# mrlooi/PoseCNN

Hardware: AMD Instinct MI355X
Metric: frames/sec 640x480x21-class Hough-vote+RoI+ADD-loss, 1/2/4/8 MI355X (higher is better)
Workload: dtype f32 (FC GEMMs: exact 3-way split-bf16 x6 MFMA, products within 2^-24, fp32 accumulate: fp32-faithful)

## Files before the change

include/posecnn_hip.h:

```cpp
#ifndef POSECNN_HIP_H
#define POSECNN_HIP_H

#include <stddef.h>
#include <stdint.h>

#ifdef __cplusplus
extern "C" {
#endif

#define PCNN_OK 0
#define PCNN_EINVAL 1
#define PCNN_EHIP 2
#define PCNN_ECAPACITY 3

#define PCNN_MAX_ROI 128

int pcnn_abi_version(void);
const char* pcnn_strerror(int code);

int pcnn_set_completion_event(void* event);
int pcnn_completion_event_pending(void);

size_t pcnn_hough_voting_workspace_size(int B, int H, int W, int C, int skip_pixels, float vote_thr);

int pcnn_hough_voting(const int32_t* label, const float* vertex, const float* extents, const float* meta,
                      int num_meta, const float* gt, int num_gt, int B, int H, int W, int C, int batch_base,
                      int global_batch, int is_train, float inlier_thr, int label_thr, float vote_thr,
                      float per_thr, int skip_pixels, float* top_box, float* top_pose, float* top_target,
                      float* top_weight, int32_t* top_domain, int32_t* num_rois, int cap, int32_t* debug_counts,
                      void* workspace, size_t workspace_bytes, void* stream);

int pcnn_hough_voting_prob(const float* prob, int32_t* label_out, const float* vertex, const float* extents,
                           const float* meta, int num_meta, const float* gt, int num_gt, int B, int H, int W, int C,
                           int batch_base, int global_batch, int is_train, float inlier_thr, int label_thr,
                           float vote_thr, float per_thr, int skip_pixels, float* top_box, float* top_pose,
                           float* top_target, float* top_weight, int32_t* top_domain, int32_t* num_rois, int cap,
                           int32_t* debug_counts, void* workspace, size_t workspace_bytes, void* stream);

int pcnn_hough_voting_compact(const int32_t* label, const float* vertex3, const float* extents, const float* meta,
                              int num_meta, const float* gt, int num_gt, int B, int H, int W, int C, int batch_base,
                              int global_batch, int is_train, float inlier_thr, int label_thr, float vote_thr,
                              float per_thr, int skip_pixels, float* top_box, float* top_pose, float* top_target,
                              float* top_weight, int32_t* top_domain, int32_t* num_rois, int cap,
                              int32_t* debug_counts, void* workspace, size_t workspace_bytes, void* stream);

int pcnn_hough_voting_grad(float* grad_label, float* grad_vertex, int B, int H, int W, int C, void* stream);

int pcnn_hough_voting_diag(const void* workspace, int B, int H, int W, int C, int skip_pixels, float vote_thr,
                           int32_t* diag_host4, void* stream);

int pcnn_roi_pool_fwd(const float* data, int B, int H, int W, int C, int layout, const float* rois, int R_cap,
                      int roi_stride, int batch_base, const int32_t* num_rois_dev, float spatial_scale, int pooled_h, int pooled_w,
                      int pool_channel, float* top, int32_t* argmax, void* stream);

int pcnn_roi_pool_fwd_accumulate(const float* data, int B, int H, int W, int C, int layout, const float* rois,
                                 int R_cap, int roi_stride, int batch_base, const int32_t* num_rois_dev,
                                 float spatial_scale, int pooled_h, int pooled_w, int pool_channel, float* top,
                                 int32_t* argmax, void* stream);

int pcnn_roi_pool_fwd_pair(const float* data_a, int Ha, int Wa, float scale_a, const float* data_b, int Hb, int Wb,
                           float scale_b, int B, int C, const float* rois, int R_cap, int roi_stride,
                           int batch_base, const int32_t* num_rois_dev, int pooled_h, int pooled_w, float* top_sum,
                           int32_t* argmax_a, int32_t* argmax_b, void* stream);

int pcnn_roi_pool_fwd_pair_px(const float* data_a, int Ha, int Wa, float scale_a, const float* data_b, int Hb,
                              int Wb, float scale_b, int B, int C, const float* rois, int R_cap, int roi_stride,
                              int batch_base, const int32_t* num_rois_dev, int pooled_h, int pooled_w,
                              float* top_sum, uint16_t* argmax_a, uint16_t* argmax_b, void* stream);

size_t pcnn_roi_pool_bwd_workspace_size(int B, int R_cap);

int pcnn_roi_pool_bwd_form(int B, int H, int W, int C, int layout, int pool_channel, int pooled_h, int pooled_w,
                           int R_cap, int px);

int pcnn_roi_pool_bwd(const float* top_diff, const int32_t* argmax, int B, int H, int W, int C, int layout,
                      const float* rois, int R_cap, int roi_stride, int batch_base, const int32_t* num_rois_dev,
                      float spatial_scale, int pooled_h, int pooled_w, int pool_channel, float* bottom_diff,
                      void* workspace, size_t workspace_bytes, void* stream);

int pcnn_roi_pool_bwd_px(const float* top_diff, const uint16_t* argmax_px, int B, int H, int W, int C,
                         const float* rois, int R_cap, int roi_stride, int batch_base, const int32_t* num_rois_dev,
                         float spatial_scale, int pooled_h, int pooled_w, float* bottom_diff, void* workspace,
                         size_t workspace_bytes, void* stream);

size_t pcnn_add_loss_workspace_size(int R_cap, int C, int P);
size_t pcnn_add_loss_stats_offset(int R_cap, int C, int P);

int pcnn_add_loss_fwd(const float* pred, const float* target, const float* weight, const float* points,
                      const float* symmetry, int R_cap, const int32_t* num_rois_dev, int C, int P, float margin,
                      int loss_norm_rows, const int32_t* loss_norm_rows_dev, float* loss, float* bottom_diff,
                      void* workspace, size_t workspace_bytes, void* stream);

int pcnn_add_loss_prep(const float* weight, const float* symmetry, int R_cap, const int32_t* num_rois_dev, int C,
                       int P, void* workspace, size_t workspace_bytes, void* stream);
int pcnn_add_loss_fwd_prepared(const float* pred, const float* target, const float* weight, const float* points,
                               const float* symmetry, int R_cap, const int32_t* num_rois_dev, int C, int P,
                               float margin, int loss_norm_rows, const int32_t* loss_norm_rows_dev, float* loss,
                               float* bottom_diff, void* workspace, size_t workspace_bytes, void* stream);

int pcnn_add_loss_fwd_head_bwd(const float* pred, const float* target, const float* weight, const float* points,
                               const float* symmetry, int R_cap, const int32_t* num_rois_dev, int C, int P,
                               float margin, int loss_norm_rows, const int32_t* loss_norm_rows_dev,
                               float* bottom_diff, void* workspace, size_t workspace_bytes, const float* tanh_out,
                               const float* d_pred_scale, float* d_y8, void* stream);
int pcnn_add_loss_total(int R_cap, const int32_t* num_rois_dev, int C, int P, const void* workspace,
                        size_t workspace_bytes, float* loss, void* stream);

int pcnn_add_loss_bwd(const float* top_diff, const float* bottom_diff, int n, const int32_t* num_rois_dev,
                      int row_len, float* out, void* stream);

int pcnn_div_rn_check(const float* x, float b, int n, int dbl, float* out, void* stream);

int pcnn_backproject_fwd(const float* data, const float* label, const float* depth, const float* meta, int num_meta,
                         const float* label_3d, int B, int H, int W, int Ch, int NC, int grid_size,
                         int kernel_size, float threshold, float* top_data, float* top_label, float* top_flag,
                         void* stream);

int pcnn_backproject_bwd(const float* top_diff, const float* depth, const float* meta, int num_meta, int B, int H,
                         int W, int Ch, int grid_size, float* bottom_diff, void* stream);

size_t pcnn_gemm_workspace_size(int M, int N, int K, int m_dynamic, int precision);

int pcnn_gemm(int M, int N, int K, const float* A, const float* A2, int lda, int a_trans, const float* B, int ldb,
              int b_trans, float* Cm, int ldc, const float* bias, int act, const float* mask, int ldm,
              const int32_t* M_dev, const int32_t* K_dev, int precision, void* workspace, size_t workspace_bytes,
              void* stream);

int pcnn_gemm_drop(int M, int N, int K, const float* A, const float* A2, int lda, int a_trans, const float* B,
                   int ldb, int b_trans, float* Cm, int ldc, const float* bias, int act, const float* mask, int ldm,
                   const uint8_t* drop, int ldd, float keep_prob, const int32_t* M_dev, const int32_t* K_dev,
                   int precision, void* workspace, size_t workspace_bytes, void* stream);

int pcnn_gemm_drop_gen(int M, int N, int K, const float* A, const float* A2, int lda, int a_trans, const float* B,
                       int ldb, int b_trans, float* Cm, int ldc, const float* bias, int act, uint8_t* drop_out,
                       int ldd, float keep_prob, uint64_t seed, const int64_t* step_dev, int stream_id,
                       const int32_t* M_dev, const int32_t* K_dev, int precision, void* workspace,
                       size_t workspace_bytes, void* stream);

size_t pcnn_tp_bytes(int rows, int K);
int pcnn_split_tp(const float* src, long row_stride, long k_stride, int rows, const int32_t* rows_dev, int K,
                  const int32_t* K_dev, void* dst, size_t dst_bytes, void* stream);
int pcnn_gemm_tp(int M, int N, int K, const void* A_tp, const void* B_tp, float* Cm, int ldc, const float* bias,
                 int act, const float* mask, int ldm, const uint8_t* drop, int ldd, float keep_prob,
                 const int32_t* M_dev, const int32_t* K_dev, void* workspace, size_t workspace_bytes, void* stream);

int pcnn_dropout_mask(uint8_t* mask, int rows, int cols, int ld, const int32_t* rows_dev, uint64_t seed,
                      const int64_t* step_dev, int stream_id, float keep_prob, void* stream);

int pcnn_philox_check(const uint32_t* ctr, const uint32_t* key, int n, uint32_t* out, void* stream);

size_t pcnn_pose2d_workspace_size(int H, int W, int C, int n_hyp);
int pcnn_pose2d(const int32_t* label, const float* vertmap, const float* extents, int H, int W, int C, float fx,
                float fy, float px, float py, uint64_t seed, int n_hyp, int max_iter, float* poses_out,
                float* hyps_out, int32_t* hyp_px, int32_t* inl_out, int32_t* final_out, void* workspace,
                size_t workspace_bytes, void* stream);

size_t pcnn_pose3d_workspace_size(int H, int W, int C, int n_hyp);
int pcnn_pose3d(const int32_t* label, const uint16_t* depth, const float* vertmap, const float* extents, int H, int W,
                int C, float fx, float fy, float px, float py, float depth_factor, uint64_t seed, int n_hyp,
                int max_iter, int nm_evals, float* poses_out, float* hyps_out, int32_t* hyp_px, int32_t* inl_out,
                int32_t* final_out, float* energy_out, float* eye_out, void* workspace, size_t workspace_bytes,
                void* stream);

int pcnn_colsum(const float* X, int M, int N, int ldx, const int32_t* M_dev, float* out, void* stream);

int pcnn_pose_head_fwd(const float* y8, const float* poses_weight, int R_cap, const int32_t* num_rois_dev, int D,
                       float* tanh_out, float* pred, void* stream);

int pcnn_pose_head_bwd(const float* d_pred, const float* d_pred_scale, const float* tanh_out,
                       const float* poses_weight, const float* pred, int R_cap, const int32_t* num_rois_dev, int D,
                       float* d_y8, void* stream);

int pcnn_box_nms(const float* rois, int R_cap, int roi_stride, const int32_t* num_rois_dev, float thresh,
                 int32_t* keep, int32_t* num_keep, const float* poses_init, const float* poses_pred, int pred_dim,
                 float* rois_out, float* poses_out, void* stream);

int pcnn_argmax_2d(const float* prob, int B, int H, int W, int C, int32_t* label, void* stream);
int pcnn_hard_label_fwd(const float* prob, const int32_t* gt, int B, int H, int W, int C, float threshold,
                        float* top, void* stream);
int pcnn_hard_label_bwd(float* grad_prob, float* grad_gt, int B, int H, int W, int C, void* stream);

int pcnn_vertex_pred_compact(const float* feat, const float* weights, const float* bias, const int32_t* label, int B,
                             int H, int W, int K, int C, float* vertex3, void* stream);

int pcnn_icp_live_vertices(const uint16_t* depth, const int32_t* label, int H, int W, const int32_t* obj_ids, int L,
                           float factor, float fx, float fy, float px, float py, float* live, void* stream);
size_t pcnn_icp_workspace_size(int N, int H, int W);
int pcnn_icp(const float* live, int num_live, const int32_t* live_index, const float* pred_vertices,
             const float* pred_normals, int N, int H, int W, float fx, float fy, float px, float py, float znear, float zfar, float max_error,
             int iterations, const float* pose_in, float* update, float* pose_out, float* systems, void* workspace,
             size_t workspace_bytes, void* stream);
size_t pcnn_icp_reduce_workspace_size(int L, int H, int W);
int pcnn_icp_center(const float* live, const int32_t* label, const int32_t* obj_ids, int L, const float* vertmap,
                    const float* pred_vertices, const float* pred_normals, int H, int W, float max_error,
                    const float* pose_in, float* out, float* pose_out, void* workspace, size_t workspace_bytes,
                    void* stream);
size_t pcnn_energy_records_workspace_size(int N, int H, int W);
int pcnn_energy_records(const float* live, int n_live, const int32_t* label, const float* pred_vertices, int H, int W,
                        float znear, float zfar, int N, const int32_t* prob_obj, const int32_t* prob_live,
                        float* records, int32_t* counts, void* workspace, size_t workspace_bytes, void* stream);
int pcnn_energy_rec(const float* records, const int32_t* counts, int stride, const float* poses,
                    const int32_t* pose_prob, int K, float znear, float zfar, float* energy, void* stream);
int pcnn_nelder_mead_energy(const float* records, const int32_t* counts, int stride, int N, const double* x0,
                            const double* lb, const double* ub, int max_eval, float znear, float zfar, double* x_out,
                            double* f_out, int32_t* nev_out, void* stream);

size_t pcnn_nelder_mead_energy_workspace_size(int N);
int pcnn_nelder_mead_energy_coop(const float* records, const int32_t* counts, int stride, int N, const double* x0,
                                 const double* lb, const double* ub, int max_eval, float znear, float zfar,
                                 double* x_out, double* f_out, int32_t* nev_out, void* workspace,
                                 size_t workspace_bytes, void* stream);
int pcnn_nelder_mead_energy_coop_path(const float* records, const int32_t* counts, int stride, int N,
                                      const double* x0, const double* lb, const double* ub, int max_eval,
                                      float znear, float zfar, double* x_out, double* f_out, int32_t* nev_out,
                                      void* workspace, size_t workspace_bytes, int force_path, int32_t* path_out,
                                      void* stream);

size_t pcnn_icp_score_workspace_size(int J, int H, int W);
int pcnn_icp_score(const float* live, const int32_t* label, int obj, const float* vertmap, int H, int W,
                   const float* hyps, int J, float radius, float* score, int32_t* choose, void* workspace,
                   size_t workspace_bytes, void* stream);
int pcnn_pose_energy(const float* live, const int32_t* label, int obj, const float* pred_vertices, int H, int W,
                     float znear, float zfar, const float* poses, int K, float* energy, void* workspace,
                     size_t workspace_bytes, void* stream);

int pcnn_pose_energy_batch(const float* live, int n_live, const int32_t* label, const float* pred_vertices, int n_pv,
                           int H, int W, float znear, float zfar, const float* poses, int K, const int32_t* pose_obj,
                           const int32_t* pose_live, const int32_t* pose_pv, float* energy, void* workspace,
                           size_t workspace_bytes, void* stream);

size_t pcnn_render_workspace_size(int K, int H, int W, int V_total, int F_max);
int pcnn_render_meshes(const float* vertices, const float* normals, const int32_t* faces, const int32_t* vert_offset,
                       const int32_t* face_offset, int M, int V_total, int F_total, int F_max,
                       const int32_t* mesh_index, const int32_t* class_id, const float* poses, int K, int H, int W,
                       float fx, float fy, float px, float py, float znear, float zfar, float* pred_vertices,
                       float* pred_normals, float* vertmap, float* depth, int32_t* tri_id, void* workspace,
                       size_t workspace_bytes, void* stream);

size_t pcnn_render_scenes_workspace_size(int S, int K, int H, int W, int V_total, int F_max);
int pcnn_render_scenes(const float* vertices, const float* normals, const int32_t* faces, const int32_t* vert_offset,
                       const int32_t* face_offset, int M, int V_total, int F_total, int F_max,
                       const int32_t* mesh_index, const int32_t* class_id, const float* poses, int K,
                       const int32_t* scene_offset, int S, int H, int W, float fx, float fy, float px, float py,
                       float znear, float zfar, int32_t* label, float* depth, float* vertmap, float* vertex3,
                       int32_t* inst_id, int32_t* visible, float* centers, void* workspace, size_t workspace_bytes,
                       void* stream);
int pcnn_vertex_targets_expand(const int32_t* label, const float* vertex3, int B, int H, int W, int C, float w_inside,
                               float* vertex_targets, float* vertex_weights, void* stream);

size_t pcnn_seg_loss_workspace_size(int B, int H, int W, int C);
int pcnn_seg_loss(const float* score, const int32_t* gt_label, int B, int H, int W, int C, float threshold,
                  float grad_scale, float* log_prob, float* prob_normalized, int32_t* label_2d,
                  float* gt_label_weight, float* d_score, float* loss, void* workspace, size_t workspace_bytes,
                  void* stream);
size_t pcnn_cross_entropy_workspace_size(int n_pix, int C);
int pcnn_cross_entropy(const float* scores, const float* labels, int n_pix, int C, float grad_scale, float* d_scores,
                       float* loss, void* workspace, size_t workspace_bytes, void* stream);
size_t pcnn_vertex_loss_workspace_size(long n);
int pcnn_vertex_loss(const float* vertex_pred, const float* vertex_targets, const float* vertex_weights, long n,
                     float sigma, float grad_scale, float* d_pred, float* loss, void* workspace,
                     size_t workspace_bytes, void* stream);
size_t pcnn_vertex_loss_compact_workspace_size(int B, int H, int W, int C);
int pcnn_vertex_loss_compact(const int32_t* label, const float* vertex3, const float* vertex_pred, int pred_ch, int B,
                             int H, int W, int C, float w_inside, float sigma, float grad_scale, float* d_pred,
                             int d_ch, float* loss, void* workspace, size_t workspace_bytes, void* stream);

size_t pcnn_vertex_pred_compact_bwd_workspace_size(int B, int H, int W, int K, int C);
int pcnn_vertex_pred_compact_bwd_partials(int B, int H, int W, int K, int C);
int pcnn_vertex_pred_compact_bwd(const float* feat, const float* weights, const int32_t* label,
                                 const float* d_vertex3, int B, int H, int W, int K, int C, float* d_feat,
                                 float* d_weights, float* d_bias, void* workspace, size_t workspace_bytes,
                                 void* stream);

#ifdef __cplusplus
}
#endif
#endif
```

posecnn_amd/_lib.py:

```python
import ctypes
import os
import threading

import torch

_HERE = os.path.dirname(os.path.abspath(__file__))
LIB_PATH = os.environ.get("POSECNN_HIP_LIB") or os.path.join(_HERE, "libposecnn_hip.so")

_lib = None
_lock = threading.Lock()

c_int = ctypes.c_int
c_float = ctypes.c_float
c_size_t = ctypes.c_size_t
c_void_p = ctypes.c_void_p

_SIGS = {
    "pcnn_abi_version": (c_int, []),
    "pcnn_strerror": (ctypes.c_char_p, [c_int]),
    "pcnn_set_completion_event": (c_int, [c_void_p]),
    "pcnn_completion_event_pending": (c_int, []),
    "pcnn_hough_voting_workspace_size": (c_size_t, [c_int, c_int, c_int, c_int, c_int, c_float]),
    "pcnn_hough_voting": (c_int, [c_void_p, c_void_p, c_void_p, c_void_p, c_int, c_void_p, c_int, c_int, c_int,
                                  c_int, c_int, c_int, c_int, c_int, c_float, c_int, c_float, c_float, c_int,
                                  c_void_p, c_void_p, c_void_p, c_void_p, c_void_p, c_void_p, c_int, c_void_p,
                                  c_void_p, c_size_t, c_void_p]),
    "pcnn_hough_voting_prob": (c_int, [c_void_p, c_void_p, c_void_p, c_void_p, c_void_p, c_int, c_void_p, c_int,
                                       c_int, c_int, c_int, c_int, c_int, c_int, c_int, c_float, c_int, c_float,
                                       c_float, c_int, c_void_p, c_void_p, c_void_p, c_void_p, c_void_p, c_void_p,
                                       c_int, c_void_p, c_void_p, c_size_t, c_void_p]),
    "pcnn_hough_voting_compact": (c_int, [c_void_p, c_void_p, c_void_p, c_void_p, c_int, c_void_p, c_int, c_int,
                                          c_int, c_int, c_int, c_int, c_int, c_int, c_float, c_int, c_float, c_float,
                                          c_int, c_void_p, c_void_p, c_void_p, c_void_p, c_void_p, c_void_p, c_int,
                                          c_void_p, c_void_p, c_size_t, c_void_p]),
    "pcnn_hough_voting_grad": (c_int, [c_void_p, c_void_p, c_int, c_int, c_int, c_int, c_void_p]),
    "pcnn_hough_voting_diag": (c_int, [c_void_p, c_int, c_int, c_int, c_int, c_int, c_float, c_void_p, c_void_p]),
    "pcnn_roi_pool_fwd": (c_int, [c_void_p, c_int, c_int, c_int, c_int, c_int, c_void_p, c_int, c_int, c_int,
                                  c_void_p, c_float, c_int, c_int, c_int, c_void_p, c_void_p, c_void_p]),
    "pcnn_roi_pool_fwd_accumulate": (c_int, [c_void_p, c_int, c_int, c_int, c_int, c_int, c_void_p, c_int, c_int,
                                             c_int, c_void_p, c_float, c_int, c_int, c_int, c_void_p, c_void_p, c_void_p]),
    "pcnn_roi_pool_fwd_pair": (c_int, [c_void_p, c_int, c_int, c_float, c_void_p, c_int, c_int, c_float, c_int, c_int,
                                       c_void_p, c_int, c_int, c_int, c_void_p, c_int, c_int, c_void_p, c_void_p,
                                       c_void_p, c_void_p]),
    "pcnn_roi_pool_fwd_pair_px": (c_int, [c_void_p, c_int, c_int, c_float, c_void_p, c_int, c_int, c_float, c_int,
                                          c_int, c_void_p, c_int, c_int, c_int, c_void_p, c_int, c_int, c_void_p,
                                          c_void_p, c_void_p, c_void_p]),
    "pcnn_roi_pool_bwd_workspace_size": (c_size_t, [c_int, c_int]),
    "pcnn_roi_pool_bwd_form": (c_int, [c_int, c_int, c_int, c_int, c_int, c_int, c_int, c_int, c_int, c_int]),
    "pcnn_roi_pool_bwd_px": (c_int, [c_void_p, c_void_p, c_int, c_int, c_int, c_int, c_void_p, c_int, c_int, c_int,
                                     c_void_p, c_float, c_int, c_int, c_void_p, c_void_p, c_size_t, c_void_p]),
    "pcnn_roi_pool_bwd": (c_int, [c_void_p, c_void_p, c_int, c_int, c_int, c_int, c_int, c_void_p, c_int, c_int,
                                  c_int, c_void_p, c_float, c_int, c_int, c_int, c_void_p, c_void_p, c_size_t, c_void_p]),
    "pcnn_add_loss_workspace_size": (c_size_t, [c_int, c_int, c_int]),
    "pcnn_add_loss_stats_offset": (c_size_t, [c_int, c_int, c_int]),
    "pcnn_add_loss_fwd": (c_int, [c_void_p, c_void_p, c_void_p, c_void_p, c_void_p, c_int, c_void_p, c_int, c_int,
                                  c_float, c_int, c_void_p, c_void_p, c_void_p, c_void_p, c_size_t, c_void_p]),
    "pcnn_add_loss_fwd_prepared": (c_int, [c_void_p, c_void_p, c_void_p, c_void_p, c_void_p, c_int, c_void_p, c_int, c_int,
                                  c_float, c_int, c_void_p, c_void_p, c_void_p, c_void_p, c_size_t, c_void_p]),
    "pcnn_add_loss_prep": (c_int, [c_void_p, c_void_p, c_int, c_void_p, c_int, c_int, c_void_p, c_size_t, c_void_p]),
    "pcnn_add_loss_fwd_head_bwd": (c_int, [c_void_p, c_void_p, c_void_p, c_void_p, c_void_p, c_int, c_void_p, c_int,
                                           c_int, c_float, c_int, c_void_p, c_void_p, c_void_p, c_size_t, c_void_p,
                                           c_void_p, c_void_p, c_void_p]),
    "pcnn_add_loss_total": (c_int, [c_int, c_void_p, c_int, c_int, c_void_p, c_size_t, c_void_p, c_void_p]),
    "pcnn_add_loss_bwd": (c_int, [c_void_p, c_void_p, c_int, c_void_p, c_int, c_void_p, c_void_p]),
    "pcnn_div_rn_check": (c_int, [c_void_p, c_float, c_int, c_int, c_void_p, c_void_p]),
    "pcnn_backproject_fwd": (c_int, [c_void_p, c_void_p, c_void_p, c_void_p, c_int, c_void_p, c_int, c_int, c_int,
                                     c_int, c_int, c_int, c_int, c_float, c_void_p, c_void_p, c_void_p, c_void_p]),
    "pcnn_backproject_bwd": (c_int, [c_void_p, c_void_p, c_void_p, c_int, c_int, c_int, c_int, c_int, c_int,
                                     c_void_p, c_void_p]),
    "pcnn_gemm_workspace_size": (c_size_t, [c_int, c_int, c_int, c_int, c_int]),
    "pcnn_gemm": (c_int, [c_int, c_int, c_int, c_void_p, c_void_p, c_int, c_int, c_void_p, c_int, c_int, c_void_p,
                          c_int, c_void_p, c_int, c_void_p, c_int, c_void_p, c_void_p, c_int, c_void_p, c_size_t,
                          c_void_p]),
    "pcnn_gemm_drop": (c_int, [c_int, c_int, c_int, c_void_p, c_void_p, c_int, c_int, c_void_p, c_int, c_int,
                               c_void_p, c_int, c_void_p, c_int, c_void_p, c_int, c_void_p, c_int, c_float, c_void_p,
                               c_void_p, c_int, c_void_p, c_size_t, c_void_p]),
    "pcnn_gemm_drop_gen": (c_int, [c_int, c_int, c_int, c_void_p, c_void_p, c_int, c_int, c_void_p, c_int, c_int,
                                   c_void_p, c_int, c_void_p, c_int, c_void_p, c_int, c_float, ctypes.c_uint64,
                                   c_void_p, c_int, c_void_p, c_void_p, c_int, c_void_p, c_size_t, c_void_p]),
    "pcnn_dropout_mask": (c_int, [c_void_p, c_int, c_int, c_int, c_void_p, ctypes.c_uint64, c_void_p, c_int, c_float,
                                  c_void_p]),
    "pcnn_philox_check": (c_int, [c_void_p, c_void_p, c_int, c_void_p, c_void_p]),
    "pcnn_pose2d_workspace_size": (c_size_t, [c_int, c_int, c_int, c_int]),
    "pcnn_pose2d": (c_int, [c_void_p, c_void_p, c_void_p, c_int, c_int, c_int, c_float, c_float, c_float, c_float,
                            ctypes.c_uint64, c_int, c_int, c_void_p, c_void_p, c_void_p, c_void_p, c_void_p, c_void_p,
                            c_size_t, c_void_p]),
    "pcnn_pose3d_workspace_size": (c_size_t, [c_int, c_int, c_int, c_int]),
    "pcnn_pose3d": (c_int, [c_void_p, c_void_p, c_void_p, c_void_p, c_int, c_int, c_int, c_float, c_float, c_float,
                            c_float, c_float, ctypes.c_uint64, c_int, c_int, c_int, c_void_p, c_void_p, c_void_p,
                            c_void_p, c_void_p, c_void_p, c_void_p, c_void_p, c_size_t, c_void_p]),
    "pcnn_tp_bytes": (c_size_t, [c_int, c_int]),
    "pcnn_split_tp": (c_int, [c_void_p, ctypes.c_long, ctypes.c_long, c_int, c_void_p, c_int, c_void_p, c_void_p,
                              c_size_t, c_void_p]),
    "pcnn_gemm_tp": (c_int, [c_int, c_int, c_int, c_void_p, c_void_p, c_void_p, c_int, c_void_p, c_int, c_void_p,
                             c_int, c_void_p, c_int, c_float, c_void_p, c_void_p, c_void_p, c_size_t, c_void_p]),
    "pcnn_colsum": (c_int, [c_void_p, c_int, c_int, c_int, c_void_p, c_void_p, c_void_p]),
    "pcnn_box_nms": (c_int, [c_void_p, c_int, c_int, c_void_p, c_float, c_void_p, c_void_p, c_void_p, c_void_p, c_int,
                             c_void_p, c_void_p, c_void_p]),
    "pcnn_argmax_2d": (c_int, [c_void_p, c_int, c_int, c_int, c_int, c_void_p, c_void_p]),
    "pcnn_hard_label_fwd": (c_int, [c_void_p, c_void_p, c_int, c_int, c_int, c_int, c_float, c_void_p, c_void_p]),
    "pcnn_hard_label_bwd": (c_int, [c_void_p, c_void_p, c_int, c_int, c_int, c_int, c_void_p]),
    "pcnn_vertex_pred_compact": (c_int, [c_void_p, c_void_p, c_void_p, c_void_p, c_int, c_int, c_int, c_int, c_int,
                                         c_void_p, c_void_p]),
    "pcnn_pose_head_fwd": (c_int, [c_void_p, c_void_p, c_int, c_void_p, c_int, c_void_p, c_void_p, c_void_p]),
    "pcnn_pose_head_bwd": (c_int, [c_void_p, c_void_p, c_void_p, c_void_p, c_void_p, c_int, c_void_p, c_int, c_void_p,
                                   c_void_p]),
    "pcnn_icp_live_vertices": (c_int, [c_void_p, c_void_p, c_int, c_int, c_void_p, c_int, c_float, c_float, c_float,
                                       c_float, c_float, c_void_p, c_void_p]),
    "pcnn_icp_workspace_size": (c_size_t, [c_int, c_int, c_int]),
    "pcnn_icp": (c_int, [c_void_p, c_int, c_void_p, c_void_p, c_void_p, c_int, c_int, c_int, c_float, c_float, c_float,
                         c_float, c_float, c_float, c_float, c_int, c_void_p, c_void_p, c_void_p, c_void_p, c_void_p,
                         c_size_t, c_void_p]),
    "pcnn_icp_reduce_workspace_size": (c_size_t, [c_int, c_int, c_int]),
    "pcnn_icp_center": (c_int, [c_void_p, c_void_p, c_void_p, c_int, c_void_p, c_void_p, c_void_p, c_int, c_int,
                                c_float, c_void_p, c_void_p, c_void_p, c_void_p, c_size_t, c_void_p]),
    "pcnn_icp_score_workspace_size": (c_size_t, [c_int, c_int, c_int]),
    "pcnn_icp_score": (c_int, [c_void_p, c_void_p, c_int, c_void_p, c_int, c_int, c_void_p, c_int, c_float, c_void_p,
                               c_void_p, c_void_p, c_size_t, c_void_p]),
    "pcnn_energy_records_workspace_size": (c_size_t, [c_int, c_int, c_int]),
    "pcnn_energy_records": (c_int, [c_void_p, c_int, c_void_p, c_void_p, c_int, c_int, c_float, c_float, c_int,
                                    c_void_p, c_void_p, c_void_p, c_void_p, c_void_p, c_size_t, c_void_p]),
    "pcnn_energy_rec": (c_int, [c_void_p, c_void_p, c_int, c_void_p, c_void_p, c_int, c_float, c_float, c_void_p,
                                c_void_p]),
    "pcnn_nelder_mead_energy": (c_int, [c_void_p, c_void_p, c_int, c_int, c_void_p, c_void_p, c_void_p, c_int,
                                        c_float, c_float, c_void_p, c_void_p, c_void_p, c_void_p]),
    "pcnn_nelder_mead_energy_workspace_size": (c_size_t, [c_int]),
    "pcnn_nelder_mead_energy_coop": (c_int, [c_void_p, c_void_p, c_int, c_int, c_void_p, c_void_p, c_void_p, c_int,
                                             c_float, c_float, c_void_p, c_void_p, c_void_p, c_void_p, c_size_t,
                                             c_void_p]),
    "pcnn_nelder_mead_energy_coop_path": (c_int, [c_void_p, c_void_p, c_int, c_int, c_void_p, c_void_p, c_void_p,
                                                  c_int, c_float, c_float, c_void_p, c_void_p, c_void_p, c_void_p,
                                                  c_size_t, c_int, c_void_p, c_void_p]),
    "pcnn_pose_energy_batch": (c_int, [c_void_p, c_int, c_void_p, c_void_p, c_int, c_int, c_int, c_float, c_float,
                                       c_void_p, c_int, c_void_p, c_void_p, c_void_p, c_void_p, c_void_p, c_size_t,
                                       c_void_p]),
    "pcnn_pose_energy": (c_int, [c_void_p, c_void_p, c_int, c_void_p, c_int, c_int, c_float, c_float, c_void_p, c_int,
                                 c_void_p, c_void_p, c_size_t, c_void_p]),
    "pcnn_render_workspace_size": (c_size_t, [c_int, c_int, c_int, c_int, c_int]),
    "pcnn_render_meshes": (c_int, [c_void_p, c_void_p, c_void_p, c_void_p, c_void_p, c_int, c_int, c_int, c_int,
                                   c_void_p, c_void_p, c_void_p, c_int, c_int, c_int, c_float, c_float, c_float,
                                   c_float, c_float, c_float, c_void_p, c_void_p, c_void_p, c_void_p, c_void_p,
                                   c_void_p, c_size_t, c_void_p]),
    "pcnn_render_scenes_workspace_size": (c_size_t, [c_int, c_int, c_int, c_int, c_int, c_int]),
    "pcnn_render_scenes": (c_int, [c_void_p, c_void_p, c_void_p, c_void_p, c_void_p, c_int, c_int, c_int, c_int,
                                   c_void_p, c_void_p, c_void_p, c_int, c_void_p, c_int, c_int, c_int, c_float,
                                   c_float, c_float, c_float, c_float, c_float, c_void_p, c_void_p, c_void_p,
                                   c_void_p, c_void_p, c_void_p, c_void_p, c_void_p, c_size_t, c_void_p]),
    "pcnn_vertex_targets_expand": (c_int, [c_void_p, c_void_p, c_int, c_int, c_int, c_int, c_float, c_void_p,
                                           c_void_p, c_void_p]),
    "pcnn_seg_loss_workspace_size": (c_size_t, [c_int, c_int, c_int, c_int]),
    "pcnn_seg_loss": (c_int, [c_void_p, c_void_p, c_int, c_int, c_int, c_int, c_float, c_float, c_void_p, c_void_p,
                              c_void_p, c_void_p, c_void_p, c_void_p, c_void_p, c_size_t, c_void_p]),
    "pcnn_cross_entropy_workspace_size": (c_size_t, [c_int, c_int]),
    "pcnn_cross_entropy": (c_int, [c_void_p, c_void_p, c_int, c_int, c_float, c_void_p, c_void_p, c_void_p, c_size_t,
                                   c_void_p]),
    "pcnn_vertex_loss_workspace_size": (c_size_t, [ctypes.c_long]),
    "pcnn_vertex_loss": (c_int, [c_void_p, c_void_p, c_void_p, ctypes.c_long, c_float, c_float, c_void_p, c_void_p,
                                 c_void_p, c_size_t, c_void_p]),
    "pcnn_vertex_loss_compact_workspace_size": (c_size_t, [c_int, c_int, c_int, c_int]),
    "pcnn_vertex_loss_compact": (c_int, [c_void_p, c_void_p, c_void_p, c_int, c_int, c_int, c_int, c_int, c_float,
                                         c_float, c_float, c_void_p, c_int, c_void_p, c_void_p, c_size_t, c_void_p]),
    "pcnn_vertex_pred_compact_bwd_workspace_size": (c_size_t, [c_int, c_int, c_int, c_int, c_int]),
    "pcnn_vertex_pred_compact_bwd_partials": (c_int, [c_int, c_int, c_int, c_int, c_int]),
    "pcnn_vertex_pred_compact_bwd": (c_int, [c_void_p, c_void_p, c_void_p, c_void_p, c_int, c_int, c_int, c_int, c_int,
                                             c_void_p, c_void_p, c_void_p, c_void_p, c_size_t, c_void_p]),
}


class PcnnError(RuntimeError):
    pass


def load():
    global _lib
    if _lib is not None:
        return _lib
    with _lock:
        if _lib is None:
            if not os.path.exists(LIB_PATH):
                raise PcnnError(f"{LIB_PATH} not built; run __graft_entry__.build() "
                                "(hipcc --offload-arch=gfx950). No CPU fallback exists.")
            lib = ctypes.CDLL(LIB_PATH)
            for name, (res, args) in _SIGS.items():
                if name.endswith("_check") and not hasattr(lib, name):
                    continue
                fn = getattr(lib, name)
                fn.restype = res
                fn.argtypes = args
            _lib = lib
    return _lib


def exported_symbols():
    return list(_SIGS.keys())


def check(rc, what):
    if rc != 0:
        msg = load().pcnn_strerror(rc).decode()
        if rc == 1:
            raise ValueError(f"{what}: {msg}")
        raise PcnnError(f"{what}: {msg} (code {rc})")


def require_gpu(*tensors):
    if not torch.cuda.is_available():
        raise PcnnError("posecnn_amd ops run only on an AMD GPU (HIP); none is visible")
    for t in tensors:
        if t is not None and not t.is_cuda:
            raise ValueError("posecnn_amd ops take device tensors (got a CPU tensor)")


class _TensorPtr(ctypes.c_void_p):
    __slots__ = ("tensor",)


def ptr(t):
    if t is None:
        return None
    p = _TensorPtr(t.data_ptr())
    p.tensor = t
    return p


def stream_ptr(stream=None):
    s = stream if stream is not None else torch.cuda.current_stream()
    return ctypes.c_void_p(s.cuda_stream)


_ws = {}


def workspace(nbytes, device, tag="default", stream=None):
    s = stream if stream is not None else torch.cuda.current_stream(device)
    key = (str(device), tag, s.cuda_stream)
    buf = _ws.get(key)
    if buf is None or buf.numel() < nbytes:
        with torch.cuda.stream(s):
            buf = torch.empty(max(int(nbytes), 256), dtype=torch.uint8, device=device)
        _ws[key] = buf
    return buf
```

posecnn_amd/build.py:

```python
import glob
import os
import subprocess
import sys
from concurrent.futures import ThreadPoolExecutor

HERE = os.path.dirname(os.path.abspath(__file__))
CSRC = os.path.join(HERE, "csrc")
OBJ = os.path.join(HERE, "build")
OUT = os.path.join(HERE, "libposecnn_hip.so")
SOURCES = ["capi.hip", "hough_compact.hip", "hough_vote.hip", "hough_peak.hip", "hough_emit.hip", "roi_pooling.hip",
           "average_distance.hip", "backprojecting.hip", "pose_head.hip", "gemm.hip", "gemm_f32.hip", "gemm_x3.hip",
           "gemm_x6.hip", "box_nms.hip", "label_producer.hip", "icp.hip", "dropout.hip", "pose2d.hip", "gemm_tp.hip",
           "render.hip", "render_scene.hip", "seg_loss.hip", "vertex_pred_bwd.hip"]
HEADERS = sorted(glob.glob(os.path.join(CSRC, "*.h"))) + [os.path.join(HERE, "..", "include", "posecnn_hip.h")]
FLAGS = ["--offload-arch=gfx950", "-O3", "-std=c++17", "-ffp-contract=off", "-fPIC", "-Wno-unused-result"]
NO_SLP = ["pose_head.hip", "gemm.hip", "gemm_f32.hip", "gemm_x3.hip", "gemm_x6.hip", "gemm_tp.hip"]
FILE_FLAGS = {src: ["-fno-slp-vectorize"] for src in NO_SLP}


def _obj(src):
    return os.path.join(OBJ, src.replace(".hip", ".o"))


def needs_build():
    if not os.path.exists(OUT):
        return True
    t = os.path.getmtime(OUT)
    deps = [os.path.join(CSRC, s) for s in SOURCES] + HEADERS + [os.path.abspath(__file__)]
    return any(os.path.getmtime(d) > t for d in deps)


def build(force=False, verbose=True):
    if not force and not needs_build():
        return OUT
    hipcc = os.environ.get("HIPCC", "/opt/rocm/bin/hipcc")
    os.makedirs(OBJ, exist_ok=True)
    newest_header = max(os.path.getmtime(h) for h in HEADERS + [os.path.abspath(__file__)])

    def compile_one(src):
        o = _obj(src)
        path = os.path.join(CSRC, src)
        if not force and os.path.exists(o) and os.path.getmtime(o) > max(os.path.getmtime(path), newest_header):
            return
        cmd = [hipcc] + FLAGS + FILE_FLAGS.get(src, []) + ["-c", path, "-o", o + ".tmp"]
        if verbose:
            print(" ".join(cmd), file=sys.stderr)
        subprocess.check_call(cmd)
        os.replace(o + ".tmp", o)

    jobs = min(len(SOURCES), max(1, min(8, os.cpu_count() or 1)))
    with ThreadPoolExecutor(jobs) as ex:
        list(ex.map(compile_one, SOURCES))
    cmd = [hipcc, "--offload-arch=gfx950", "-shared", "-fPIC", "-o", OUT + ".tmp"] + [_obj(s) for s in SOURCES]
    if verbose:
        print(" ".join(cmd), file=sys.stderr)
    subprocess.check_call(cmd)
    os.replace(OUT + ".tmp", OUT)
    return OUT


if __name__ == "__main__":
    build(force="--force" in sys.argv)
```

posecnn_amd/csrc/gemm.hip:

```cpp
#include "gemm_common.h"
#include "pcnn_philox.h"

using namespace pcnn_gk;

namespace {

__device__ __forceinline__ float drop_gen_epi(float v, const GemmArgs& g, uint32_t step, int m, int n) {
  const uint32_t q = pcnn_philox::keep_quad((uint64_t)m * (uint64_t)(g.N >> 2) + (uint64_t)(n >> 2), g.drop_k0,
                                            g.drop_k1, g.drop_sid, step, g.keep);
  if ((n & 3) == 0) *(uint32_t*)((uint8_t*)g.drop + (size_t)m * g.ldd + n) = q;
  if (g.keep != 1.f) v = v / g.keep;
  return v * (float)((q >> (8 * (n & 3))) & 1u);
}

__global__ void __launch_bounds__(256) k_gemm_reduce(GemmArgs g) {
  const int Meff = eff_dim(g.M, g.M_dev);
  const int Keff = eff_dim(g.K, g.K_dev);
  const int S = g.prec ? x_plan(Meff, g.N, Keff, g.tile, g.xgrid, split_bk(g.prec)).S : split_for(Meff, g.N, Keff);
  const bool dr = g.drop || g.keep != 1.f;
  const uint32_t step = g.drop_gen && g.drop_step ? (uint32_t)*g.drop_step : 0u;
  auto dropv = [&](float v, int m, int n) { return g.drop_gen ? drop_gen_epi(v, g, step, m, n) : drop_epi(v, g, m, n); };
  if (S == 1) {
    if (!dr || keep_in_epilogue(g)) return;
    const long total = (long)Meff * g.N;
    for (long i = (long)blockIdx.x * blockDim.x + threadIdx.x; i < total; i += (long)gridDim.x * blockDim.x) {
      const int m = (int)(i / g.N), n = (int)(i % g.N);
      float* c = g.C + (size_t)m * g.ldc + n;
      *c = dropv(*c, m, n);
    }
    return;
  }
  const size_t slab_stride = (size_t)g.M * g.N;
  const bool vec = (long)g.M * g.N < (1l << 31) && (g.N & 3) == 0 && (g.ldc & 3) == 0 && (!g.mask || (g.ldm & 3) == 0) &&
                   (!g.drop || (g.ldd & 3) == 0) &&
                   ((((uintptr_t)g.slab) | ((uintptr_t)g.C) | ((uintptr_t)g.mask) | ((uintptr_t)g.bias)) & 15) == 0;
  if (vec) {
    const int n4 = g.N >> 2;
    const int total4 = Meff * n4;
    for (int i = blockIdx.x * blockDim.x + threadIdx.x; i < total4; i += gridDim.x * blockDim.x) {
      const int m = i / n4, n = (i - m * n4) << 2;
      const float4* sp = (const float4*)(g.slab + (size_t)m * g.N + n);
      float4 v = sp[0];
      for (int z = 1; z < S; z++) {
        const float4 t = sp[z * (slab_stride >> 2)];
        v.x += t.x; v.y += t.y; v.z += t.z; v.w += t.w;
      }
      float4 o = make_float4(epilogue(v.x, g, m, n), epilogue(v.y, g, m, n + 1), epilogue(v.z, g, m, n + 2),
                             epilogue(v.w, g, m, n + 3));
      if (g.drop_gen) {
        const uint32_t q = pcnn_philox::keep_quad((uint64_t)i, g.drop_k0, g.drop_k1, g.drop_sid, step, g.keep);
        *(uint32_t*)((uint8_t*)g.drop + (size_t)m * g.ldd + n) = q;
        o = make_float4((g.keep != 1.f ? o.x / g.keep : o.x) * (float)(q & 1u),
                        (g.keep != 1.f ? o.y / g.keep : o.y) * (float)((q >> 8) & 1u),
                        (g.keep != 1.f ? o.z / g.keep : o.z) * (float)((q >> 16) & 1u),
                        (g.keep != 1.f ? o.w / g.keep : o.w) * (float)((q >> 24) & 1u));
      } else if (dr) {
        o = make_float4(drop_epi(o.x, g, m, n), drop_epi(o.y, g, m, n + 1), drop_epi(o.z, g, m, n + 2),
                        drop_epi(o.w, g, m, n + 3));
      }
      *(float4*)(g.C + (size_t)m * g.ldc + n) = o;
    }
    return;
  }
  const long total = (long)Meff * g.N;
  for (long i = (long)blockIdx.x * blockDim.x + threadIdx.x; i < total; i += (long)gridDim.x * blockDim.x) {
    const int m = (int)(i / g.N), n = (int)(i % g.N);
    float v = 0.f;
    for (int z = 0; z < S; z++) v += g.slab[((size_t)z * g.M + m) * g.N + n];
    v = epilogue(v, g, m, n);
    g.C[(size_t)m * g.ldc + n] = dr ? dropv(v, m, n) : v;
  }
}

}

namespace pcnn_gk {
void launch_gemm_reduce(const GemmArgs& g, hipStream_t st) {
  hipLaunchKernelGGL(k_gemm_reduce, dim3(1024), dim3(256), 0, st, g);
}
}

extern "C" size_t pcnn_gemm_workspace_size(int M, int N, int K, int m_dynamic, int precision) {
  return gemm_workspace_bytes(M, N, K, m_dynamic != 0, precision);
}

extern "C" int pcnn_gemm(int M, int N, int K, const float* A, const float* A2, int lda, int a_trans, const float* B,
                         int ldb, int b_trans, float* Cm, int ldc, const float* bias, int act, const float* mask,
                         int ldm, const int32_t* M_dev, const int32_t* K_dev, int precision, void* workspace,
                         size_t workspace_bytes, void* stream) {
  return pcnn_gemm_drop(M, N, K, A, A2, lda, a_trans, B, ldb, b_trans, Cm, ldc, bias, act, mask, ldm, nullptr, 0, 1.f,
                        M_dev, K_dev, precision, workspace, workspace_bytes, stream);
}

static int gemm_impl(int M, int N, int K, const float* A, const float* A2, int lda, int a_trans, const float* B,
                     int ldb, int b_trans, float* Cm, int ldc, const float* bias, int act, const float* mask, int ldm,
                     const uint8_t* drop, int ldd, float keep_prob, const int32_t* M_dev, const int32_t* K_dev,
                     int precision, void* workspace, size_t workspace_bytes, void* stream, int drop_gen,
                     uint64_t seed, const int64_t* step_dev, int stream_id) {
  PCNN_REQUIRE(M >= 0 && N > 0 && K >= 0 && A && B && Cm);
  PCNN_REQUIRE(!drop_gen || (drop && N % 4 == 0 && ldd % 4 == 0 && ((uintptr_t)drop & 3) == 0 && stream_id >= 0 &&
                             (long)M * (N / 4) < (1l << 31)));
  PCNN_REQUIRE(keep_prob > 0.f && keep_prob <= 1.f);
  PCNN_REQUIRE(!drop || (ldd >= N && (long)M * ldd < (1l << 31)));
  PCNN_REQUIRE(precision >= 0 && precision <= 2);
  PCNN_REQUIRE(lda >= (a_trans ? M : K) && ldb >= (b_trans ? K : N) && ldc >= N);
  PCNN_REQUIRE(!mask || ldm >= N);
  PCNN_REQUIRE(act == 0 || act == 1);
  PCNN_REQUIRE(precision == 0 || (lda % 4 == 0 && ldb % 4 == 0 && ((uintptr_t)A & 15) == 0 &&
                                  ((uintptr_t)B & 15) == 0 && (!A2 || ((uintptr_t)A2 & 15) == 0)));
  PCNN_REQUIRE(precision == 0 || ((long)(a_trans ? K : M) * lda < (1l << 29) && (long)(b_trans ? N : K) * ldb < (1l << 29) &&
                                  (long)M * ldc < (1l << 29) && (!mask || (long)M * ldm < (1l << 29))));
  if (M == 0) return PCNN_OK;
  if (workspace_bytes < pcnn_gemm_workspace_size(M, N, K, M_dev != nullptr, precision) || !workspace)
    return PCNN_ECAPACITY;
  const LaunchPlan plan = plan_launch(M, N, K, M_dev != nullptr, precision);
  GemmArgs g{M, N, K, A, A2, lda, B, ldb, Cm, ldc, bias, act, mask, ldm, M_dev, K_dev, (float*)workspace, precision,
             plan.tile, plan.grid, plan.c_stream, drop, ldd, keep_prob};
  if (drop_gen) {
    g.drop_gen = 1;
    g.drop_k0 = (uint32_t)seed;
    g.drop_k1 = (uint32_t)(seed >> 32);
    g.drop_sid = (uint32_t)stream_id;
    g.drop_step = step_dev;
  }
  hipStream_t st = (hipStream_t)stream;
  const bool reduce_after = reduce_follows(plan, precision, drop, keep_prob);
  if (precision == 0) {
    launch_gemm_f32(g, a_trans, b_trans, st);
    if (reduce_after) launch_gemm_reduce(g, st);
    PCNN_CHECK_LAUNCH();
    return PCNN_OK;
  }
  const bool a_kc = !a_trans, b_kc = b_trans;
  const bool ragged = ((a_kc || b_kc) && (K % 4 != 0 || K_dev != nullptr)) || (!a_kc && M % 4 != 0) ||
                      (!b_kc && N % 4 != 0);
  const SplitVariant v{a_trans != 0, b_trans != 0, ragged, A2 != nullptr, plan.gen};
  const hipEvent_t done_ev = reduce_after ? pcnn::take_done_event() : nullptr;
  if (precision == 2) launch_gemm_x6(g, v, st);
  else launch_gemm_x3(g, v, st);
  if (reduce_after) {
    pcnn::t_done_event = done_ev;
    pcnn::launch_last(k_gemm_reduce, dim3(1024), dim3(256), 0, st, g);
  }
  PCNN_CHECK_LAUNCH();
  return PCNN_OK;
}

extern "C" int pcnn_gemm_drop(int M, int N, int K, const float* A, const float* A2, int lda, int a_trans,
                              const float* B, int ldb, int b_trans, float* Cm, int ldc, const float* bias, int act,
                              const float* mask, int ldm, const uint8_t* drop, int ldd, float keep_prob,
                              const int32_t* M_dev, const int32_t* K_dev, int precision, void* workspace,
                              size_t workspace_bytes, void* stream) {
  return gemm_impl(M, N, K, A, A2, lda, a_trans, B, ldb, b_trans, Cm, ldc, bias, act, mask, ldm, drop, ldd, keep_prob,
                   M_dev, K_dev, precision, workspace, workspace_bytes, stream, 0, 0, nullptr, 0);
}

extern "C" int pcnn_gemm_drop_gen(int M, int N, int K, const float* A, const float* A2, int lda, int a_trans,
                                  const float* B, int ldb, int b_trans, float* Cm, int ldc, const float* bias, int act,
                                  uint8_t* drop_out, int ldd, float keep_prob, uint64_t seed,
                                  const int64_t* step_dev, int stream_id, const int32_t* M_dev, const int32_t* K_dev,
                                  int precision, void* workspace, size_t workspace_bytes, void* stream) {
  return gemm_impl(M, N, K, A, A2, lda, a_trans, B, ldb, b_trans, Cm, ldc, bias, act, nullptr, 0, drop_out, ldd,
                   keep_prob, M_dev, K_dev, precision, workspace, workspace_bytes, stream, 1, seed, step_dev,
                   stream_id);
}
```

posecnn_amd/csrc/head_common.h:

```cpp
#pragma once
#include "pcnn_common.h"

namespace pcnn_head {

__device__ __forceinline__ void head_bwd_row(const float (&dp)[4], const float* __restrict__ t_in,
                                             const float* __restrict__ pw, const float* __restrict__ pred, int row,
                                             int D, int lane, float* __restrict__ dy8) {
  float ss = 0.f, dot = 0.f;
#pragma unroll
  for (int k = 0; k < 4; k++) {
    const int c = lane + 64 * k;
    if (c < D) {
      const float mv = t_in[(size_t)row * D + c] * pw[(size_t)row * D + c];
      ss += mv * mv;
      dot += pred[(size_t)row * D + c] * dp[k];
    }
  }
  ss = pcnn::wave_sum(ss);
  dot = pcnn::wave_sum(dot);
  const bool clamp = !(ss > 1e-12f);
  const float inv = 1.f / sqrtf(fmaxf(ss, 1e-12f));
#pragma unroll
  for (int k = 0; k < 4; k++) {
    const int c = lane + 64 * k;
    if (c < D) {
      const size_t o = (size_t)row * D + c;
      const float dm = clamp ? dp[k] * inv : (dp[k] - pred[o] * dot) * inv;
      const float dt = dm * pw[o];
      const float t = t_in[o];
      dy8[o] = dt * (1.f - t * t);
    }
  }
}

}
```

posecnn_amd/csrc/pose_head.hip:

```cpp
#include "gemm_common.h"
#include "head_common.h"
#include <math.h>

using namespace pcnn_gk;

namespace {

__global__ void __launch_bounds__(1024) k_colsum(const float* __restrict__ X, int M, int N, int ldx,
                                                 const int32_t* __restrict__ M_dev, float* __restrict__ out) {
  __shared__ float part[16][65];
  const int Meff = eff_dim(M, M_dev);
  const int col = threadIdx.x & 63, grp = threadIdx.x >> 6;
  const int n = blockIdx.x * 64 + col;
  float s = 0.f;
  if (n < N)
    for (int m = grp; m < Meff; m += 16) s += X[(size_t)m * ldx + n];
  part[grp][col] = s;
  __syncthreads();
  if (grp == 0 && n < N) {
    float t = 0.f;
    for (int g = 0; g < 16; g++) t += part[g][col];
    out[n] = t;
  }
}

__global__ void __launch_bounds__(256) k_head_fwd(const float* __restrict__ y8, const float* __restrict__ pw,
                                                   int R_cap, const int32_t* __restrict__ num_rois_dev, int D,
                                                   float* __restrict__ t_out, float* __restrict__ pred) {
  const int R = eff_dim(R_cap, num_rois_dev);
  const int row = (blockIdx.x * blockDim.x + threadIdx.x) >> 6;
  const int lane = pcnn::lane_id();
  if (row >= R) return;
  float mv[4];
  float ss = 0.f;
#pragma unroll
  for (int k = 0; k < 4; k++) {
    const int c = lane + 64 * k;
    mv[k] = 0.f;
    if (c < D) {
      const float t = tanhf(y8[(size_t)row * D + c]);
      t_out[(size_t)row * D + c] = t;
      mv[k] = t * pw[(size_t)row * D + c];
      ss += mv[k] * mv[k];
    }
  }
  ss = pcnn::wave_sum(ss);
  const float inv = 1.f / sqrtf(fmaxf(ss, 1e-12f));
#pragma unroll
  for (int k = 0; k < 4; k++) {
    const int c = lane + 64 * k;
    if (c < D) pred[(size_t)row * D + c] = mv[k] * inv;
  }
}

__global__ void __launch_bounds__(256) k_head_bwd(const float* __restrict__ dpred, const float* __restrict__ t_in,
                                                   const float* __restrict__ pw, const float* __restrict__ pred,
                                                   int R_cap, const int32_t* __restrict__ num_rois_dev, int D,
                                                   const float* __restrict__ dscale, float* __restrict__ dy8) {
  const int R = eff_dim(R_cap, num_rois_dev);
  const float g = dscale ? dscale[0] : 1.f;
  const int row = (blockIdx.x * blockDim.x + threadIdx.x) >> 6;
  const int lane = pcnn::lane_id();
  if (row >= R) return;
  float dp[4];
#pragma unroll
  for (int k = 0; k < 4; k++) {
    const int c = lane + 64 * k;
    dp[k] = c < D ? g * dpred[(size_t)row * D + c] : 0.f;
  }
  pcnn_head::head_bwd_row(dp, t_in, pw, pred, row, D, lane, dy8);
}

}

extern "C" int pcnn_colsum(const float* X, int M, int N, int ldx, const int32_t* M_dev, float* out, void* stream) {
  PCNN_REQUIRE(X && out && M >= 0 && N > 0 && ldx >= N);
  hipLaunchKernelGGL(k_colsum, dim3((N + 63) / 64), dim3(1024), 0, (hipStream_t)stream, X, M, N, ldx, M_dev, out);
  PCNN_CHECK_LAUNCH();
  return PCNN_OK;
}

extern "C" int pcnn_pose_head_fwd(const float* y8, const float* poses_weight, int R_cap, const int32_t* num_rois_dev,
                                  int D, float* tanh_out, float* pred, void* stream) {
  PCNN_REQUIRE(y8 && poses_weight && tanh_out && pred && R_cap >= 0 && D > 0 && D <= 256);
  if (R_cap == 0) return PCNN_OK;
  hipLaunchKernelGGL(k_head_fwd, dim3((R_cap + 3) / 4), dim3(256), 0, (hipStream_t)stream, y8, poses_weight, R_cap,
                     num_rois_dev, D, tanh_out, pred);
  PCNN_CHECK_LAUNCH();
  return PCNN_OK;
}

extern "C" int pcnn_pose_head_bwd(const float* d_pred, const float* d_pred_scale, const float* tanh_out,
                                  const float* poses_weight, const float* pred, int R_cap,
                                  const int32_t* num_rois_dev, int D, float* d_y8, void* stream) {
  PCNN_REQUIRE(d_pred && tanh_out && poses_weight && pred && d_y8 && R_cap >= 0 && D > 0 && D <= 256);
  if (R_cap == 0) return PCNN_OK;
  hipLaunchKernelGGL(k_head_bwd, dim3((R_cap + 3) / 4), dim3(256), 0, (hipStream_t)stream, d_pred, tanh_out,
                     poses_weight, pred, R_cap, num_rois_dev, D, d_pred_scale, d_y8);
  PCNN_CHECK_LAUNCH();
  return PCNN_OK;
}
```

posecnn_amd/pipeline.py:

```python
import contextlib

import torch

from . import _lib
from . import pose_head as ph
from .hough_voting_gpu_layer import hough_voting_gpu_op as hv
from .roi_pooling_layer import roi_pooling_op as rp
from .average_distance_loss import average_distance_loss_op as adl
from .exchange import GradShard, RoiExchange

CAP = hv.CAPACITY
_nullctx = contextlib.nullcontext


class PoseStep:
    def __init__(self, B, H, W, num_classes, device, conv4_hw=None, conv5_hw=None, channels=512, units=4096,
                 is_train=1, skip_pixels=10, vote_threshold=-1.0, vote_percentage=0.02, margin=0.01,
                 global_batch=None, batch_base=0, weights=None, dist=None, backward=True, precision=2,
                 overlap_weight_grads=True, pixel_argmax=True, keep_prob=None, drop_seed=0x5EED, side_prep=True,
                 drop_in_reduce=True, pipeline=False, prefetch_at="loss", fuse_loss_tail=True,
                 defer_side_join=False, signal_forks=True, pool_at_tail=False):
        self.B, self.H, self.W, self.C = B, H, W, num_classes
        self.dev = device
        self.is_train, self.skip, self.vthr, self.vper, self.margin = is_train, skip_pixels, vote_threshold, \
            vote_percentage, margin
        self.global_batch = global_batch or B
        self.batch_base = batch_base
        self.dist = dist
        self.backward = backward
        self.prec = precision
        self.h4, self.w4 = conv4_hw or (H // 8, W // 8)
        self.h5, self.w5 = conv5_hw or (H // 16, W // 16)
        self.Ch = channels
        D = 4 * num_classes
        self.D = D
        self.weights = weights or ph.PoseHeadWeights(num_classes, device, in_dim=49 * channels, units=units)
        f32 = dict(dtype=torch.float32, device=device)
        i32 = dict(dtype=torch.int32, device=device)
        K6 = 49 * channels
        px = pixel_argmax and max(self.h4 * self.w4, self.h5 * self.w5) < 0xFFFF
        adt = dict(dtype=torch.int16 if px else torch.int32, device=device)

        def minibatch_set():
            return dict(hough=dict(box=torch.zeros((CAP, 7), **f32), pose=torch.zeros((CAP, 7), **f32),
                                   target=torch.zeros((CAP, D), **f32), weight=torch.zeros((CAP, D), **f32),
                                   domain=torch.zeros((CAP,), **i32), num_rois=torch.zeros((2,), **i32)),
                        pool=torch.zeros((CAP, 7, 7, channels), **f32),
                        arg5=torch.zeros((CAP, 7, 7, channels), **adt),
                        arg4=torch.zeros((CAP, 7, 7, channels), **adt),
                        add_ws=None, prepped=False)
        self.fuse_loss_tail = fuse_loss_tail
        self.pipeline = bool(pipeline)
        self._sets = [minibatch_set() for _ in range(2 if self.pipeline else 1)]
        self._cur = 0
        self._primed = None
        self.prefetch_at = prefetch_at
        if prefetch_at not in ("loss", "bwd", "start", "fwd", "tail"):
            raise ValueError("prefetch_at must be 'start', 'fwd', 'loss', 'bwd' or 'tail'")
        self._fork_ev = torch.cuda.Event() if self.pipeline else None
        self._fork_recorded = False
        self.pre_stream = torch.cuda.Stream(device=device) if self.pipeline else None
        self._next = None
        self.y6 = torch.zeros((CAP, units), **f32)
        self.y7 = torch.zeros((CAP, units), **f32)
        self.y8 = torch.zeros((CAP, D), **f32)
        self.t8 = torch.zeros((CAP, D), **f32)
        self.pred = torch.zeros((CAP, D), **f32)
        self.loss = torch.zeros((1,), **f32)
        self.diff = torch.zeros((CAP, D), **f32)
        self.one = torch.ones((1,), **f32)
        self.dy8 = torch.zeros((CAP, D), **f32)
        self.dy7 = torch.zeros((CAP, units), **f32)
        self.dy6 = torch.zeros((CAP, units), **f32)
        self.dx = torch.zeros((CAP, K6), **f32)
        self.gshard = None
        if dist is not None:
            per_max = 9 if is_train else 1
            slot = max(1, min(CAP, B * (hv.MAX_ROI // self.global_batch) * per_max))
            self.gshard = GradShard(dist, slot, [("w6", (K6, units)), ("w7", (units, units)), ("w8", (units, D))],
                                    device)
        self.grads = self.weights.grads_like()
        if self.gshard is not None:
            for k in ("w6", "w7", "w8"):
                self.grads[k] = self.grads[k][self.gshard.rows(k)].contiguous()
        self.keep = float(keep_prob if keep_prob is not None else (0.5 if is_train else 1.0))
        if not 0.0 < self.keep <= 1.0:
            raise ValueError("keep_prob must be in (0, 1]")
        self.drop6 = self.drop7 = None
        self._drop_external = False
        self.drop_in_reduce = drop_in_reduce
        self._bump_drop_step = False
        self._drawn = False
        if self.keep < 1.0:
            u8 = dict(dtype=torch.uint8, device=device)
            self.drop6 = torch.zeros((CAP, units), **u8)
            self.drop7 = torch.zeros((CAP, units), **u8)
            self.drop_step = torch.zeros((1,), dtype=torch.int64, device=device)
            rank = dist.get_rank() if dist is not None else 0
            self.drop_seed = (int(drop_seed) + rank * 0x9E3779B97F4A7C15) & ((1 << 64) - 1)
            self._drop_ready = None
            self._drop_ev = torch.cuda.Event()
        self.dconv4 = torch.zeros((B, self.h4, self.w4, channels), **f32)
        self.dconv5 = torch.zeros((B, self.h5, self.w5, channels), **f32)
        self.norm_rows = torch.zeros((1,), **i32)
        self.timer = None
        self.gemm_timer = None
        self.xchg = None
        self.detections = None
        self._pending = {}
        self._in_step = False
        self.side_stream = torch.cuda.Stream(device=device) if overlap_weight_grads else None
        self.side_prep = side_prep and self.side_stream is not None
        self.defer_side_join = bool(defer_side_join) and self.pipeline and dist is None and \
            self.side_stream is not None
        self._side_mid_ev = torch.cuda.Event() if self.defer_side_join else None
        self._side_done_ev = torch.cuda.Event() if self.defer_side_join else None
        self._side_pending = False
        self.signal_forks = bool(signal_forks) and self.side_stream is not None and dist is None
        self._fork_evs = {}
        self.pool_at_tail = bool(pool_at_tail) and self.pipeline
        self._pool_pending = None
        if self.signal_forks:
            for k in ("loss", "fc8_dx", "fc7_dx"):
                ev = torch.cuda.Event()
                ev.record()
                self._fork_evs[k] = ev
        self._mid_covers_pre = False
        self._mid_waited = False

    def _t(self, name):
        step = self

        class _Ctx:
            def __enter__(self_):
                if step.timer is not None:
                    self_.e0 = torch.cuda.Event(enable_timing=True)
                    self_.e0.record()

            def __exit__(self_, *a):
                if step.timer is not None:
                    e1 = torch.cuda.Event(enable_timing=True)
                    e1.record()
                    step.timer.setdefault(name, []).append((self_.e0, e1))
        return _Ctx()

    def join(self):
        cur = torch.cuda.current_stream()
        for st in (self.side_stream, self.pre_stream):
            if st is not None:
                cur.wait_stream(st)
        self._side_pending = False

    def _side_wait(self, ev_name, stream=None):
        if self._side_pending:
            (stream or torch.cuda.current_stream()).wait_event(getattr(self, ev_name))

    def _arm_fork(self, name):
        if not self.signal_forks or self.timer is not None or torch.cuda.is_current_stream_capturing():
            return None
        ev = self._fork_evs[name]
        _lib.load().pcnn_set_completion_event(ev.cuda_event)
        return ev

    @staticmethod
    def _fork_taken(ev):
        if ev is None:
            return None
        return None if _lib.load().pcnn_completion_event_pending() else ev

    def _fork_side(self, side, ev):
        if ev is not None:
            side.wait_event(ev)
        else:
            side.wait_stream(torch.cuda.current_stream())

    hough = property(lambda self: self._sets[self._cur]["hough"])
    pool = property(lambda self: self._sets[self._cur]["pool"])
    arg5 = property(lambda self: self._sets[self._cur]["arg5"])
    arg4 = property(lambda self: self._sets[self._cur]["arg4"])
    add_ws = property(lambda self: self._sets[self._cur]["add_ws"])

    def vote(self, label, vertex, extents, meta, gt, s=None):
        s = self._cur if s is None else s
        self._sets[s]["pooled"] = False
        with self._t("hough_voting_gpu"):
            return hv.hough_voting_gpu_capacity(label, vertex, extents, meta, gt, self.is_train, self.vthr,
                                                self.vper, self.skip, global_batch=self.global_batch,
                                                batch_base=self.batch_base, out=self._sets[s]["hough"])

    def add_prep(self, points, symmetry, s=None, stream=None):
        s = self._cur if s is None else s
        st = self._sets[s]
        if st["add_ws"] is None:
            st["add_ws"] = torch.empty(adl.workspace_bytes(CAP, self.C, points.shape[1]), dtype=torch.uint8,
                                       device=self.dev)
        h = st["hough"]
        side = None
        if stream is None:
            side = self.side_stream if self.timer is None and self.side_prep else None
            if side is not None:
                side.wait_stream(torch.cuda.current_stream())
        with torch.cuda.stream(stream or side or torch.cuda.current_stream()):
            adl.average_distance_loss_prep(h["weight"], symmetry, points.shape[1], st["add_ws"],
                                           num_rois=h["num_rois"][1:2])
        st["prepped"] = "side" if side is not None else "stream"

    def pool_fwd(self, conv4, conv5, s=None):
        s = self._cur if s is None else s
        st = self._sets[s]
        with self._t("roi_pool_fwd"):
            rp.roi_pool_pair(conv5, 1.0 / 16.0, conv4, 1.0 / 8.0, st["hough"]["box"], 7, 7,
                             num_rois=st["hough"]["num_rois"][1:2], out=(st["pool"], st["arg5"], st["arg4"]),
                             batch_base=self.batch_base)
        st["pooled"] = True

    def _front(self, inputs, s, stream=None):
        ctx = torch.cuda.stream(stream) if stream is not None else _nullctx()
        with ctx:
            self.vote(inputs["label"], inputs["vertex"], inputs["extents"], inputs["meta"], inputs["gt"], s=s)
            if stream is not None:
                self.add_prep(inputs["points"], inputs["symmetry"], s=s, stream=stream)
                if self.pool_at_tail and stream is self.pre_stream:
                    self._pool_pending = (inputs, s)
                else:
                    self.pool_fwd(inputs["conv4"], inputs["conv5"], s=s)

    def _issue_pending_pool(self):
        if self._pool_pending is None:
            return
        inputs, s = self._pool_pending
        self._pool_pending = None
        with torch.cuda.stream(self.pre_stream):
            self.pool_fwd(inputs["conv4"], inputs["conv5"], s=s)

    def _prefetch(self):
        if self._next is None:
            return
        nxt, s = self._next
        self._next = None
        if self.timer is not None:
            self._side_wait("_side_done_ev")
            self._side_pending = False
            self._front(nxt, s, stream=torch.cuda.current_stream())
        else:
            if self._fork_recorded:
                self.pre_stream.wait_event(self._fork_ev)
            else:
                self.pre_stream.wait_stream(torch.cuda.current_stream())
            self._side_wait("_side_done_ev", self.pre_stream)
            self._front(nxt, s, stream=self.pre_stream)
        self._fork_recorded = False
        self._primed = (s, nxt)

    def set_drop_masks(self, m6, m7):
        if self.keep >= 1.0:
            raise ValueError("set_drop_masks: the step has keep_prob 1 (no dropout)")
        for dst, m in ((self.drop6, m6), (self.drop7, m7)):
            dst.zero_()
            dst[:m.shape[0]].copy_(m.to(torch.uint8))
        self._drop_external = True

    def draw_drop_masks(self):
        if self.keep >= 1.0 or self._drop_external or self.drop_in_reduce:
            return
        self._drawn = True
        nr = self.hough["num_rois"][1:2]
        side = self.side_stream if self.timer is None and self.side_prep else None
        if side is not None:
            side.wait_stream(torch.cuda.current_stream())
        with torch.cuda.stream(side or torch.cuda.current_stream()):
            ph.dropout_mask(self.drop6, self.keep, self.drop_seed, self.drop_step, 6, rows_dev=nr)
            ph.dropout_mask(self.drop7, self.keep, self.drop_seed, self.drop_step, 7, rows_dev=nr)
            self.drop_step.add_(1)
            if side is not None:
                self._drop_ev.record(side)
                self._drop_ready = self._drop_ev

    def exchange(self):
        h = self.hough
        if self.dist is None:
            self.norm_rows = h["num_rois"][1:2]
            return
        with self._t("allreduce_rows"):
            self.norm_rows.copy_(h["num_rois"][0:1])
            self._pending["rows"] = self.dist.all_reduce(self.norm_rows, async_op=True)

    def _wait(self, key):
        w = self._pending.pop(key, None)
        if w is not None:
            w.wait()

    def gather_detections(self):
        h = self.hough
        if self.dist is None:
            return torch.cat([h["box"], h["pose"]], 1), h["num_rois"][0:1]
        return self._exchange_rows()(h["box"], h["pose"], h["num_rois"])

    def _exchange_rows(self):
        if self.xchg is None:
            self.xchg = RoiExchange(self.dist, CAP, self.dev)
        return self.xchg

    def forward(self, conv4, conv5, points, symmetry):
        h = self.hough
        nr = h["num_rois"][1:2]
        w = self.weights
        K6 = 49 * self.Ch
        st = self._sets[self._cur]
        if not (self.pipeline and st.get("pooled")):
            self.pool_fwd(conv4, conv5)
        x = self.pool.view(CAP, K6)
        gs = self.gshard if self.backward else None
        if gs is not None:
            gs.send_input("w6", x)
        dk = dict(keep_prob=self.keep) if self.keep < 1.0 else {}
        if not self._drawn:
            self.draw_drop_masks()
        self._drawn = False
        if self.keep < 1.0 and getattr(self, "_drop_ready", None) is not None:
            torch.cuda.current_stream().wait_event(self._drop_ready)
            self._drop_ready = None
        gen = self.keep < 1.0 and self.drop_in_reduce and not self._drop_external
        g6 = dict(drop_gen=(self.drop_seed, self.drop_step, 6)) if gen else {}
        g7 = dict(drop_gen=(self.drop_seed, self.drop_step, 7)) if gen else {}
        if not self._mid_waited:
            self._side_wait("_side_mid_ev")
        self._mid_waited = False
        with self._t("gemm_fc6_fwd"):
            self._g("fc6_fwd", x, w.w6, self.y6, bias=w.b6, act=1, M_dev=nr, drop=self.drop6, **dk, **g6)
        if self.prefetch_at == "fwd":
            self._prefetch()
        if gs is not None:
            gs.send_input("w7", self.y6)
        with self._t("gemm_fc7_fc8_fwd"):
            self._g("fc7_fwd", self.y6, w.w7, self.y7, bias=w.b7, act=1, M_dev=nr, drop=self.drop7, **dk, **g7)
            if gs is not None:
                gs.send_input("w8", self.y7)
            self._g("fc8_fwd", self.y7, w.w8, self.y8, bias=w.b8, act=0, M_dev=nr)
        if self.prefetch_at == "loss":
            self._prefetch()
        if gen:
            if self._in_step and self.backward:
                self._bump_drop_step = True
            else:
                self.drop_step.add_(1)
        if self.dist is not None:
            self._wait("rows")
            self.norm_rows.clamp_(min=1)
        with self._t("head_add_loss_fwd"):
            ph.head_fwd(self.y8, h["weight"], self.t8, self.pred, num_rois=nr)
            if not st["prepped"]:
                self.add_prep(points, symmetry)
            if st["prepped"] == "side":
                torch.cuda.current_stream().wait_stream(self.side_stream)
            st["prepped"] = False
            self._wait("loss")
            side = self.side_stream
            self._head_bwd_done = fuse = (self.fuse_loss_tail and self._in_step and self.backward and
                                          self.timer is None and side is not None and self.D <= 256)
            if fuse:
                ev = self._arm_fork("loss")
                adl.average_distance_loss_head_bwd(self.pred, h["target"], h["weight"], points, symmetry,
                                                   self.margin, self.t8, self.one, self.diff, self.dy8, st["add_ws"],
                                                   num_rois=nr, loss_norm_rows_dev=self.norm_rows)
                self._fork_side(side, self._fork_taken(ev))
                with torch.cuda.stream(side):
                    adl.average_distance_loss_total(CAP, self.C, points.shape[1], st["add_ws"], self.loss,
                                                    num_rois=nr)
                    if self.dist is not None:
                        self._pending["loss"] = self.dist.all_reduce(self.loss, async_op=True)
                return self.loss
            adl.average_distance_loss(self.pred, h["target"], h["weight"], points, symmetry, self.margin,
                                      num_rois=nr, loss_norm_rows_dev=self.norm_rows, out=(self.loss, self.diff),
                                      workspace=st["add_ws"], prepared=True)
        if self.dist is not None:
            self._pending["loss"] = self.dist.all_reduce(self.loss, async_op=True)
            if not self._in_step:
                self._wait("loss")
        return self.loss

    def backward_pass(self, conv4, conv5):
        h = self.hough
        nr = h["num_rois"][1:2]
        w, g = self.weights, self.grads
        K6 = 49 * self.Ch
        main = torch.cuda.current_stream()
        side = self.side_stream if self.timer is None else None
        gs = self.gshard
        x = self.pool.view(CAP, K6)

        def weight_grads(name, X, dY, K_loc, M, N, fork=True, fork_ev=None):
            if side is not None and fork:
                self._fork_side(side, fork_ev)
            if gs is not None:
                gs.send_grad(name, dY, nr)
            with torch.cuda.stream(side or main):
                if gs is not None:
                    gs.reduce(name, g[name], g["b" + name[1:]],
                              lambda A, B_, C_, **kw: self._g(f"fc{name[1:]}_dw", A, B_, C_, **kw), ph.colsum)
                else:
                    ph.colsum(dY, g["b" + name[1:]], M_dev=nr)
                    self._g(f"fc{name[1:]}_dw", X, dY, g[name], a_trans=1, K_dev=nr, M=M, N=N, K=K_loc)

        fused_fork = getattr(self, "_head_bwd_done", False) and side is not None
        if not getattr(self, "_head_bwd_done", False):
            with self._t("add_loss_head_bwd"):
                ph.head_bwd(self.diff, self.t8, h["weight"], self.pred, self.dy8, num_rois=nr,
                            d_pred_scale=self.one)
        self._head_bwd_done = False
        if self.prefetch_at == "bwd":
            self._prefetch()
        with self._t("gemm_fc8_fc7_dw_bias"):
            weight_grads("w8", self.y7, self.dy8, CAP, w.units, self.D, fork=not fused_fork)
        dk = dict(keep_prob=self.keep) if self.keep < 1.0 else {}
        ev = self._arm_fork("fc8_dx") if side is not None else None
        with self._t("gemm_fc8_fc7_dx"):
            self._g("fc8_dx", self.dy8, w.w8, self.dy7, b_trans=1, mask=self.y7, M_dev=nr, **dk)
        ev = self._fork_taken(ev)
        with self._t("gemm_fc8_fc7_dw_bias"):
            weight_grads("w7", self.y6, self.dy7, CAP, w.units, w.units, fork_ev=ev)
        defer = self.defer_side_join and side is not None
        self._side_wait("_side_done_ev")
        self._side_pending = False
        if defer:
            self._mid_covers_pre = (self._primed is not None and self._pool_pending is None and
                                    not torch.cuda.is_current_stream_capturing())
            if self._mid_covers_pre:
                side.wait_stream(self.pre_stream)
            if self._bump_drop_step and self._mid_covers_pre:
                with torch.cuda.stream(side):
                    self.drop_step.add_(1)
                self._bump_drop_step = False
            self._side_mid_ev.record(side)
        ev = self._arm_fork("fc7_dx") if side is not None else None
        with self._t("gemm_fc8_fc7_dx"):
            self._g("fc7_dx", self.dy7, w.w7, self.dy6, b_trans=1, mask=self.y6, M_dev=nr, **dk)
        ev = self._fork_taken(ev)
        with self._t("gemm_fc6_dw"):
            weight_grads("w6", x, self.dy6, CAP, K6, w.units, fork_ev=ev)
        with self._t("gemm_fc6_dx"):
            self._g("fc6_dx", self.dy6, w.w6, self.dx, b_trans=1, M_dev=nr)
        if self.prefetch_at == "tail":
            self._prefetch()
        self._issue_pending_pool()
        dxp = self.dx.view(CAP, 7, 7, self.Ch)
        with self._t("roi_pool_bwd"):
            rp.roi_pool_grad(conv5, h["box"], self.arg5, dxp, 7, 7, 1.0 / 16.0, 0, num_rois=nr, out=self.dconv5,
                             batch_base=self.batch_base)
            rp.roi_pool_grad(conv4, h["box"], self.arg4, dxp, 7, 7, 1.0 / 8.0, 0, num_rois=nr, out=self.dconv4,
                             batch_base=self.batch_base)
        if self._bump_drop_step:
            self.drop_step.add_(1)
            self._bump_drop_step = False
        if defer:
            self._side_done_ev.record(side)
            self._side_pending = True
        elif side is not None:
            main.wait_stream(side)

    def _g(self, name, A, B, C, **kw):
        if self.gemm_timer is None:
            return ph.gemm(A, B, C, precision=self.prec, **kw)
        e0, e1 = torch.cuda.Event(enable_timing=True), torch.cuda.Event(enable_timing=True)
        e0.record()
        ph.gemm(A, B, C, precision=self.prec, **kw)
        e1.record()
        self.gemm_timer.setdefault(name, []).append((e0, e1))
        return C

    def step(self, inputs, next_inputs=None):
        if self.pipeline:
            return self._step_pipelined(inputs, next_inputs)
        if next_inputs is not None:
            raise ValueError("next_inputs needs PoseStep(pipeline=True)")
        self.vote(inputs["label"], inputs["vertex"], inputs["extents"], inputs["meta"], inputs["gt"])
        self.draw_drop_masks()
        if self.side_prep:
            self.add_prep(inputs["points"], inputs["symmetry"])
        return self._train(inputs)

    def _step_pipelined(self, inputs, next_inputs):
        main = torch.cuda.current_stream()
        if self._primed is not None and self._primed[1] is inputs:
            self._cur = self._primed[0]
            if self._side_pending and self._mid_covers_pre:
                main.wait_event(self._side_mid_ev)
                self._mid_waited = True
            else:
                main.wait_stream(self.pre_stream)
        else:
            self._side_wait("_side_done_ev")
            self._side_pending = False
            self._front(inputs, self._cur, stream=main)
        self._primed = None
        self._next = (next_inputs, 1 - self._cur) if next_inputs is not None else None
        self.draw_drop_masks()
        if self.prefetch_at == "start":
            self._prefetch()
        elif self.prefetch_at == "fwd" and self._next is not None and self.timer is None:
            self._fork_ev.record(main)
            self._fork_recorded = True
        loss = self._train(inputs)
        self._prefetch()
        self._issue_pending_pool()
        return loss

    def _train(self, inputs):
        self.exchange()
        if self.dist is not None:
            with self._t("allgather_rois"):
                h = self.hough
                self._exchange_rows().start(h["box"], h["pose"], h["num_rois"])
        self._in_step = True
        try:
            loss = self.forward(inputs["conv4"], inputs["conv5"], inputs["points"], inputs["symmetry"])
            if self.backward:
                self.backward_pass(inputs["conv4"], inputs["conv5"])
        finally:
            self._in_step = False
        self._wait("loss")
        if self.dist is not None:
            rows, total = self.xchg.finish()
            self.detections = (rows.clone(), total.clone())
        return loss
```

posecnn_amd/pose_head.py:

```python
import torch

from . import _lib


def gemm(A, B, C, a_trans=0, b_trans=0, A2=None, bias=None, act=0, mask=None, M_dev=None, K_dev=None, M=None,
         N=None, K=None, precision=2, drop=None, keep_prob=1.0, drop_gen=None, stream=None):
    _lib.require_gpu(A, B, C)
    for t in (A, B, C, A2, bias, mask):
        if t is not None and (t.dtype != torch.float32 or t.stride(-1) != 1):
            raise ValueError("gemm operands must be fp32 with unit inner stride")
    if drop is not None and (drop.dtype != torch.uint8 or drop.stride(-1) != 1 or not drop.is_cuda):
        raise ValueError("gemm: drop must be a uint8 device tensor with unit inner stride")
    if M is None:
        M = A.shape[1] if a_trans else A.shape[0]
    if K is None:
        K = A.shape[0] if a_trans else A.shape[1]
    if N is None:
        N = B.shape[0] if b_trans else B.shape[1]
    lib = _lib.load()
    ws = _lib.workspace(lib.pcnn_gemm_workspace_size(M, N, K, int(M_dev is not None), precision), C.device, "gemm",
                        stream)
    if drop_gen is not None:
        if drop is None or mask is not None:
            raise ValueError("gemm: drop_gen needs the drop output buffer and no mask (forward only)")
        seed, step_dev, sid = drop_gen
        if step_dev is not None and (step_dev.dtype != torch.int64 or not step_dev.is_cuda):
            raise ValueError("gemm: drop_gen's step counter must be an int64 device tensor")
        rc = lib.pcnn_gemm_drop_gen(M, N, K, _lib.ptr(A), _lib.ptr(A2), A.stride(0), int(a_trans), _lib.ptr(B),
                                    B.stride(0), int(b_trans), _lib.ptr(C), C.stride(0), _lib.ptr(bias), int(act),
                                    _lib.ptr(drop), drop.stride(0), float(keep_prob), int(seed) & ((1 << 64) - 1),
                                    _lib.ptr(step_dev), int(sid), _lib.ptr(M_dev), _lib.ptr(K_dev), int(precision),
                                    _lib.ptr(ws), ws.numel(), _lib.stream_ptr(stream))
    elif drop is None and keep_prob == 1.0:
        rc = lib.pcnn_gemm(M, N, K, _lib.ptr(A), _lib.ptr(A2), A.stride(0), int(a_trans), _lib.ptr(B), B.stride(0),
                           int(b_trans), _lib.ptr(C), C.stride(0), _lib.ptr(bias), int(act), _lib.ptr(mask),
                           mask.stride(0) if mask is not None else 0, _lib.ptr(M_dev), _lib.ptr(K_dev),
                           int(precision), _lib.ptr(ws), ws.numel(), _lib.stream_ptr(stream))
    else:
        rc = lib.pcnn_gemm_drop(M, N, K, _lib.ptr(A), _lib.ptr(A2), A.stride(0), int(a_trans), _lib.ptr(B),
                                B.stride(0), int(b_trans), _lib.ptr(C), C.stride(0), _lib.ptr(bias), int(act),
                                _lib.ptr(mask), mask.stride(0) if mask is not None else 0, _lib.ptr(drop),
                                drop.stride(0) if drop is not None else 0, float(keep_prob), _lib.ptr(M_dev),
                                _lib.ptr(K_dev), int(precision), _lib.ptr(ws), ws.numel(), _lib.stream_ptr(stream))
    _lib.check(rc, "gemm")
    return C


def tp_bytes(rows, K):
    return int(_lib.load().pcnn_tp_bytes(int(rows), int(K)))


def split_tp(src, rows, K, out, row_stride, k_stride, rows_dev=None, K_dev=None, stream=None):
    _lib.require_gpu(src, out)
    if src.dtype != torch.float32 or out.dtype != torch.uint8 or not out.is_contiguous():
        raise ValueError("split_tp: fp32 source, contiguous uint8 destination")
    rc = _lib.load().pcnn_split_tp(_lib.ptr(src), int(row_stride), int(k_stride), int(rows), _lib.ptr(rows_dev),
                                   int(K), _lib.ptr(K_dev), _lib.ptr(out), out.numel(), _lib.stream_ptr(stream))
    _lib.check(rc, "split_tp")
    return out


def gemm_tp(A_tp, B_tp, C, M, N, K, bias=None, act=0, mask=None, drop=None, keep_prob=1.0, M_dev=None, K_dev=None,
            stream=None):
    _lib.require_gpu(A_tp, B_tp, C)
    for t in (C, bias, mask):
        if t is not None and (t.dtype != torch.float32 or t.stride(-1) != 1):
            raise ValueError("gemm_tp: fp32 outputs / epilogue operands with unit inner stride")
    if drop is not None and (drop.dtype != torch.uint8 or drop.stride(-1) != 1):
        raise ValueError("gemm_tp: drop must be uint8 with unit inner stride")
    lib = _lib.load()
    ws = _lib.workspace(lib.pcnn_gemm_workspace_size(M, N, K, int(M_dev is not None), 2), C.device, "gemm", stream)
    rc = lib.pcnn_gemm_tp(int(M), int(N), int(K), _lib.ptr(A_tp), _lib.ptr(B_tp), _lib.ptr(C), C.stride(0),
                          _lib.ptr(bias), int(act), _lib.ptr(mask), mask.stride(0) if mask is not None else 0,
                          _lib.ptr(drop), drop.stride(0) if drop is not None else 0, float(keep_prob),
                          _lib.ptr(M_dev), _lib.ptr(K_dev), _lib.ptr(ws), ws.numel(), _lib.stream_ptr(stream))
    _lib.check(rc, "gemm_tp")
    return C


def dropout_mask(mask, keep_prob, seed, step_dev=None, stream_id=0, rows_dev=None, stream=None):
    _lib.require_gpu(mask)
    if mask.dtype != torch.uint8 or mask.dim() != 2 or mask.stride(1) != 1:
        raise ValueError("dropout_mask: uint8 (rows, cols) mask with unit inner stride")
    if step_dev is not None and (step_dev.dtype != torch.int64 or not step_dev.is_cuda):
        raise ValueError("dropout_mask: step_dev must be an int64 device tensor")
    rc = _lib.load().pcnn_dropout_mask(_lib.ptr(mask), mask.shape[0], mask.shape[1], mask.stride(0),
                                       _lib.ptr(rows_dev), int(seed) & ((1 << 64) - 1), _lib.ptr(step_dev),
                                       int(stream_id), float(keep_prob), _lib.stream_ptr(stream))
    _lib.check(rc, "dropout_mask")
    return mask


def colsum(X, out, M_dev=None, stream=None):
    rc = _lib.load().pcnn_colsum(_lib.ptr(X), X.shape[0], X.shape[1], X.stride(0), _lib.ptr(M_dev), _lib.ptr(out),
                                 _lib.stream_ptr(stream))
    _lib.check(rc, "colsum")
    return out


def head_fwd(y8, poses_weight, tanh_out, pred, num_rois=None, stream=None):
    R, D = y8.shape
    rc = _lib.load().pcnn_pose_head_fwd(_lib.ptr(y8), _lib.ptr(poses_weight), R, _lib.ptr(num_rois), D,
                                        _lib.ptr(tanh_out), _lib.ptr(pred), _lib.stream_ptr(stream))
    _lib.check(rc, "pose_head_fwd")


def head_bwd(d_pred, tanh_out, poses_weight, pred, d_y8, num_rois=None, d_pred_scale=None, stream=None):
    R, D = d_pred.shape
    rc = _lib.load().pcnn_pose_head_bwd(_lib.ptr(d_pred), _lib.ptr(d_pred_scale), _lib.ptr(tanh_out),
                                        _lib.ptr(poses_weight), _lib.ptr(pred), R, _lib.ptr(num_rois), D,
                                        _lib.ptr(d_y8), _lib.stream_ptr(stream))
    _lib.check(rc, "pose_head_bwd")


def truncated_normal(shape, std, generator, device):
    t = torch.empty(shape, dtype=torch.float32, device=device)
    torch.nn.init.trunc_normal_(t, 0.0, std, -2 * std, 2 * std, generator=generator)
    return t


class PoseHeadWeights:

    def __init__(self, num_classes, device, in_dim=7 * 7 * 512, units=4096, seed=0):
        g = torch.Generator(device=device)
        g.manual_seed(seed)
        D = 4 * num_classes
        self.w6 = truncated_normal((in_dim, units), 0.001, g, device)
        self.b6 = torch.zeros(units, device=device)
        self.w7 = truncated_normal((units, units), 0.001, g, device)
        self.b7 = torch.zeros(units, device=device)
        self.w8 = truncated_normal((units, D), 0.001, g, device)
        self.b8 = torch.zeros(D, device=device)
        self.in_dim, self.units, self.D = in_dim, units, D

    def grads_like(self):
        return {k: torch.empty_like(getattr(self, k)) for k in ("w6", "b6", "w7", "b7", "w8", "b8")}
```

Before: 4639.

## Fuse fc7 split-K reduction and epilogue into fc8 GEMM; add skinny fc8 dx kernel

Adds a fused path where fc7 writes only its split-K partial slabs, and a new fc8 kernel reduces those slabs, applies the bias/ReLU/dropout epilogue, writes y7 and the dropout mask, and feeds the tile straight into a 6-MFMA split-bf16 fc8 GEMM through LDS. A second kernel reduces the fc8 partials, adds b8 and runs the pose head forward in the same pass. A dedicated skinny kernel handles the fc8 input-gradient GEMM with the mask and keep scaling applied in its epilogue. The aim is to cut separate reduce/epilogue launches and round trips of the fc7 activations through global memory. In exchange it adds a lot of new kernel code and depends on the workspace layout shared with the existing GEMM planner.

```diff
diff --git a/include/posecnn_hip.h b/include/posecnn_hip.h
--- a/include/posecnn_hip.h
+++ b/include/posecnn_hip.h
@@ -170,6 +170,20 @@
 int pcnn_pose_head_bwd(const float* d_pred, const float* d_pred_scale, const float* tanh_out,
                        const float* poses_weight, const float* pred, int R_cap, const int32_t* num_rois_dev, int D,
                        float* d_y8, void* stream);
+
+int pcnn_gemm_partial(int M, int N, int K, const float* A, const float* A2, int lda, int a_trans, const float* B,
+                      int ldb, int b_trans, float* Cm, int ldc, const float* bias, int act, const int32_t* M_dev,
+                      const int32_t* K_dev, int precision, void* workspace, size_t workspace_bytes, void* stream);
+int pcnn_fc8_fwd_fused(int M, int N7, int K7, const void* fc7_workspace, size_t fc7_workspace_bytes, const float* b7,
+                       int act7, float* y7, int ld7, uint8_t* drop, int ldd, float keep_prob, int drop_gen,
+                       uint64_t seed, const int64_t* step_dev, int stream_id, const float* W8, int ldb, int D,
+                       const int32_t* M_dev, void* fc8_workspace, size_t fc8_workspace_bytes, void* stream);
+int pcnn_fc8_reduce_head_fwd(const void* fc8_workspace, size_t fc8_workspace_bytes, const float* b8, int R_cap, int K,
+                             int D, const int32_t* num_rois_dev, const float* poses_weight, float* y8,
+                             float* tanh_out, float* pred, void* stream);
+int pcnn_fc8_dx_skinny(const float* dy8, int lda, const float* W8, int ldb, const float* mask, int ldm,
+                       float keep_prob, float* dy7, int ldc, int M, int D, int N7, const int32_t* M_dev,
+                       void* stream);
 
 int pcnn_box_nms(const float* rois, int R_cap, int roi_stride, const int32_t* num_rois_dev, float thresh,
                  int32_t* keep, int32_t* num_keep, const float* poses_init, const float* poses_pred, int pred_dim,
diff --git a/posecnn_amd/_lib.py b/posecnn_amd/_lib.py
--- a/posecnn_amd/_lib.py
+++ b/posecnn_amd/_lib.py
@@ -102,6 +102,16 @@
     "pcnn_hard_label_bwd": (c_int, [c_void_p, c_void_p, c_int, c_int, c_int, c_int, c_void_p]),
     "pcnn_vertex_pred_compact": (c_int, [c_void_p, c_void_p, c_void_p, c_void_p, c_int, c_int, c_int, c_int, c_int,
                                          c_void_p, c_void_p]),
+    "pcnn_gemm_partial": (c_int, [c_int, c_int, c_int, c_void_p, c_void_p, c_int, c_int, c_void_p, c_int, c_int,
+                                  c_void_p, c_int, c_void_p, c_int, c_void_p, c_void_p, c_int, c_void_p, c_size_t,
+                                  c_void_p]),
+    "pcnn_fc8_fwd_fused": (c_int, [c_int, c_int, c_int, c_void_p, c_size_t, c_void_p, c_int, c_void_p, c_int, c_void_p,
+                                   c_int, c_float, c_int, ctypes.c_uint64, c_void_p, c_int, c_void_p, c_int, c_int,
+                                   c_void_p, c_void_p, c_size_t, c_void_p]),
+    "pcnn_fc8_reduce_head_fwd": (c_int, [c_void_p, c_size_t, c_void_p, c_int, c_int, c_int, c_void_p, c_void_p,
+                                         c_void_p, c_void_p, c_void_p, c_void_p]),
+    "pcnn_fc8_dx_skinny": (c_int, [c_void_p, c_int, c_void_p, c_int, c_void_p, c_int, c_float, c_void_p, c_int, c_int,
+                                   c_int, c_int, c_void_p, c_void_p]),
     "pcnn_pose_head_fwd": (c_int, [c_void_p, c_void_p, c_int, c_void_p, c_int, c_void_p, c_void_p, c_void_p]),
     "pcnn_pose_head_bwd": (c_int, [c_void_p, c_void_p, c_void_p, c_void_p, c_void_p, c_int, c_void_p, c_int, c_void_p,
                                    c_void_p]),
diff --git a/posecnn_amd/build.py b/posecnn_amd/build.py
--- a/posecnn_amd/build.py
+++ b/posecnn_amd/build.py
@@ -11,10 +11,11 @@
 SOURCES = ["capi.hip", "hough_compact.hip", "hough_vote.hip", "hough_peak.hip", "hough_emit.hip", "roi_pooling.hip",
            "average_distance.hip", "backprojecting.hip", "pose_head.hip", "gemm.hip", "gemm_f32.hip", "gemm_x3.hip",
            "gemm_x6.hip", "box_nms.hip", "label_producer.hip", "icp.hip", "dropout.hip", "pose2d.hip", "gemm_tp.hip",
-           "render.hip", "render_scene.hip", "seg_loss.hip", "vertex_pred_bwd.hip"]
+           "render.hip", "render_scene.hip", "seg_loss.hip", "vertex_pred_bwd.hip", "fc8_fused.hip"]
 HEADERS = sorted(glob.glob(os.path.join(CSRC, "*.h"))) + [os.path.join(HERE, "..", "include", "posecnn_hip.h")]
 FLAGS = ["--offload-arch=gfx950", "-O3", "-std=c++17", "-ffp-contract=off", "-fPIC", "-Wno-unused-result"]
-NO_SLP = ["pose_head.hip", "gemm.hip", "gemm_f32.hip", "gemm_x3.hip", "gemm_x6.hip", "gemm_tp.hip"]
+NO_SLP = ["pose_head.hip", "gemm.hip", "gemm_f32.hip", "gemm_x3.hip", "gemm_x6.hip", "gemm_tp.hip",
+          "fc8_fused.hip"]
 FILE_FLAGS = {src: ["-fno-slp-vectorize"] for src in NO_SLP}
 
 
diff --git a/posecnn_amd/csrc/fc8_fused.hip b/posecnn_amd/csrc/fc8_fused.hip
--- /dev/null
+++ b/posecnn_amd/csrc/fc8_fused.hip
@@ -0,0 +1,389 @@
+#include "gemm_common.h"
+#include "head_common.h"
+#include "pcnn_philox.h"
+
+using namespace pcnn_gk;
+
+namespace {
+
+typedef unsigned u32x4 __attribute__((ext_vector_type(4)));
+
+constexpr int F8BK = 16;
+constexpr int F8CH = 8;
+constexpr int F8ROW = F8CH * F8BK * 2 + 16;
+constexpr int F8PLANE = 32 * F8ROW;
+constexpr int F8MAXD = 128;
+
+__device__ __forceinline__ int f8_qrow(int q) { return (q & 3) + 8 * (q >> 2); }
+
+__device__ __forceinline__ void f8_split8(const float (&v)[8], bf16x8& hi, bf16x8& mid, bf16x8& lo) {
+  u32x4 h, m, l;
+#pragma unroll
+  for (int p = 0; p < 4; p++) {
+    unsigned a, b, c;
+    x_split3(v[2 * p], v[2 * p + 1], a, b, c);
+    h[p] = a;
+    m[p] = b;
+    l[p] = c;
+  }
+  hi = __builtin_bit_cast(bf16x8, h);
+  mid = __builtin_bit_cast(bf16x8, m);
+  lo = __builtin_bit_cast(bf16x8, l);
+}
+
+__device__ __forceinline__ f32x16 f8_mfma6(bf16x8 ah, bf16x8 am, bf16x8 al, bf16x8 bh, bf16x8 bm, bf16x8 bl,
+                                           f32x16 acc) {
+  acc = __builtin_amdgcn_mfma_f32_32x32x16_bf16(al, bh, acc, 0, 0, 0);
+  acc = __builtin_amdgcn_mfma_f32_32x32x16_bf16(ah, bl, acc, 0, 0, 0);
+  acc = __builtin_amdgcn_mfma_f32_32x32x16_bf16(am, bm, acc, 0, 0, 0);
+  acc = __builtin_amdgcn_mfma_f32_32x32x16_bf16(am, bh, acc, 0, 0, 0);
+  acc = __builtin_amdgcn_mfma_f32_32x32x16_bf16(ah, bm, acc, 0, 0, 0);
+  acc = __builtin_amdgcn_mfma_f32_32x32x16_bf16(ah, bh, acc, 0, 0, 0);
+  return acc;
+}
+
+struct Fc8Fwd {
+  const float* W8;
+  int ldb, D;
+  int tile8, grid8;
+  float* slab8;
+};
+
+__global__ void __launch_bounds__(256, 2) k_fc8_fwd_fused(GemmArgs g, Fc8Fwd a) {
+  __shared__ __attribute__((aligned(16))) char xl[3 * F8PLANE];
+  const int Meff = eff_dim(g.M, g.M_dev);
+  const int K8 = g.N;
+  const int S7 = x_plan(Meff, g.N, eff_dim(g.K, g.K_dev), g.tile, g.xgrid, split_bk(g.prec)).S;
+  const XPlan p8 = x_plan(Meff, a.D, K8, a.tile8, a.grid8, F8BK);
+  const int kstep = (p8.ns + p8.S - 1) / p8.S;
+  const int mb = (Meff + 31) / 32;
+  const int items = mb * p8.S;
+  const int t = threadIdx.x, lane = pcnn::lane_id(), wave = t >> 6;
+  const int r = lane & 31, hsel = lane >> 5;
+  const bool mm = wave * 32 < a.D;
+  const bool dr = g.drop || g.keep != 1.f;
+  const uint32_t step = g.drop_gen && g.drop_step ? (uint32_t)*g.drop_step : 0u;
+  const int n4 = g.N >> 2;
+  const size_t slab_stride = (size_t)g.M * g.N;
+  const XOp oc = x_op(g.C, g.ldc, (long)(g.M - 1) * g.ldc + g.N);
+  const XOp ow = x_op(a.W8, a.ldb, (long)(K8 - 1) * a.ldb + a.D);
+  const int ncol = wave * 32 + r;
+
+  for (int item = blockIdx.x; item < items; item += gridDim.x) {
+    const int z = item / mb, m0 = (item - z * mb) * 32;
+    const int kl = z * kstep, kh = min(p8.ns, kl + kstep);
+    const int nsteps = kh > kl ? kh - kl : 0;
+    f32x16 acc = (f32x16){};
+    for (int c0 = 0; c0 < nsteps; c0 += F8CH) {
+      const int nch = min(F8CH, nsteps - c0);
+      const int kb = (kl + c0) * F8BK, ke = min(K8, kb + nch * F8BK);
+      unsigned vo[4];
+      bool ok[4];
+      xf4 v[4];
+#pragma unroll
+      for (int u = 0; u < 4; u++) {
+        const int qi = t + 256 * u;
+        const int m = m0 + (qi >> 5), n = kb + 4 * (qi & 31);
+        ok[u] = m < Meff && n < ke;
+        vo[u] = ok[u] ? (unsigned)(m * g.N + n) * 4u : kXOob;
+      }
+      if (S7 == 1) {
+#pragma unroll
+        for (int u = 0; u < 4; u++) {
+          const int qi = t + 256 * u;
+          const int m = m0 + (qi >> 5), n = kb + 4 * (qi & 31);
+          v[u] = x_ld4(oc, ok[u] ? (unsigned)(m * g.ldc + n) * 4u : kXOob, 0);
+        }
+      } else {
+        const XOp o0 = x_op(g.slab, g.N, (long)slab_stride);
+#pragma unroll
+        for (int u = 0; u < 4; u++) v[u] = x_ld4(o0, vo[u], 0);
+        int zz = 1;
+        for (; zz + 7 <= S7; zz += 7) {
+          xf4 tt[7][4];
+#pragma unroll
+          for (int d = 0; d < 7; d++) {
+            const XOp oz = x_op(g.slab + (zz + d) * slab_stride, g.N, (long)slab_stride);
+#pragma unroll
+            for (int u = 0; u < 4; u++) tt[d][u] = x_ld4(oz, vo[u], 0);
+          }
+#pragma unroll
+          for (int d = 0; d < 7; d++)
+#pragma unroll
+            for (int u = 0; u < 4; u++) {
+              v[u][0] += tt[d][u][0]; v[u][1] += tt[d][u][1]; v[u][2] += tt[d][u][2]; v[u][3] += tt[d][u][3];
+            }
+        }
+        for (; zz < S7; zz++) {
+          const XOp oz = x_op(g.slab + zz * slab_stride, g.N, (long)slab_stride);
+#pragma unroll
+          for (int u = 0; u < 4; u++) {
+            const xf4 tt = x_ld4(oz, vo[u], 0);
+            v[u][0] += tt[0]; v[u][1] += tt[1]; v[u][2] += tt[2]; v[u][3] += tt[3];
+          }
+        }
+      }
+      float bv[F8CH][8];
+#pragma unroll
+      for (int s = 0; s < F8CH; s++)
+#pragma unroll
+        for (int e = 0; e < 8; e++) {
+          const int k = kb + F8BK * s + 8 * hsel + e;
+          const bool okb = mm && ncol < a.D && k < ke;
+          bv[s][e] = x_ld1(ow, okb ? (unsigned)(k * a.ldb + ncol) * 4u : kXOob, 0);
+        }
+#pragma unroll
+      for (int u = 0; u < 4; u++) {
+        const int qi = t + 256 * u;
+        const int row = qi >> 5, kq = qi & 31;
+        const int m = m0 + row, n = kb + 4 * kq;
+        float4 o = make_float4(0.f, 0.f, 0.f, 0.f);
+        if (ok[u]) {
+          o = make_float4(v[u][0], v[u][1], v[u][2], v[u][3]);
+          if (S7 != 1)
+            o = make_float4(epilogue(o.x, g, m, n), epilogue(o.y, g, m, n + 1), epilogue(o.z, g, m, n + 2),
+                            epilogue(o.w, g, m, n + 3));
+          if (g.drop_gen) {
+            const uint32_t q = pcnn_philox::keep_quad((uint64_t)(m * n4 + (n >> 2)), g.drop_k0, g.drop_k1, g.drop_sid,
+                                                      step, g.keep);
+            *(uint32_t*)((uint8_t*)g.drop + (size_t)m * g.ldd + n) = q;
+            o = make_float4((g.keep != 1.f ? o.x / g.keep : o.x) * (float)(q & 1u),
+                            (g.keep != 1.f ? o.y / g.keep : o.y) * (float)((q >> 8) & 1u),
+                            (g.keep != 1.f ? o.z / g.keep : o.z) * (float)((q >> 16) & 1u),
+                            (g.keep != 1.f ? o.w / g.keep : o.w) * (float)((q >> 24) & 1u));
+          } else if (dr) {
+            o = make_float4(drop_epi(o.x, g, m, n), drop_epi(o.y, g, m, n + 1), drop_epi(o.z, g, m, n + 2),
+                            drop_epi(o.w, g, m, n + 3));
+          }
+          if (S7 != 1 || dr) *(float4*)(g.C + (size_t)m * g.ldc + n) = o;
+        }
+        unsigned h0, m0_, l0, h1, m1, l1;
+        x_split3(o.x, o.y, h0, m0_, l0);
+        x_split3(o.z, o.w, h1, m1, l1);
+        char* p = xl + row * F8ROW + 8 * kq;
+        *(uint2*)p = make_uint2(h0, h1);
+        *(uint2*)(p + F8PLANE) = make_uint2(m0_, m1);
+        *(uint2*)(p + 2 * F8PLANE) = make_uint2(l0, l1);
+      }
+      __syncthreads();
+      if (mm) {
+#pragma unroll
+        for (int s = 0; s < F8CH; s++)
+          if (s < nch) {
+            const char* p = xl + r * F8ROW + 2 * (F8BK * s + 8 * hsel);
+            const bf16x8 ah = *(const bf16x8*)p;
+            const bf16x8 am = *(const bf16x8*)(p + F8PLANE);
+            const bf16x8 al = *(const bf16x8*)(p + 2 * F8PLANE);
+            bf16x8 bh, bm, bl;
+            f8_split8(bv[s], bh, bm, bl);
+            acc = f8_mfma6(ah, am, al, bh, bm, bl, acc);
+          }
+      }
+      __syncthreads();
+    }
+    if (mm && ncol < a.D) {
+#pragma unroll
+      for (int q = 0; q < 16; q++) {
+        const int m = m0 + 4 * hsel + f8_qrow(q);
+        const float vq = acc[q];
+        if (m < Meff) a.slab8[((size_t)z * g.M + m) * a.D + ncol] = vq;
+      }
+    }
+  }
+}
+
+__global__ void __launch_bounds__(256) k_fc8_reduce_head_fwd(const float* __restrict__ slab,
+                                                              const float* __restrict__ b8, int M, int K, int D,
+                                                              int tile8, int grid8, int vec,
+                                                              const int32_t* __restrict__ M_dev,
+                                                              const float* __restrict__ pw, float* __restrict__ y8,
+                                                              float* __restrict__ t_out, float* __restrict__ pred) {
+  const int R = eff_dim(M, M_dev);
+  const int row = (blockIdx.x * blockDim.x + threadIdx.x) >> 6;
+  const int lane = pcnn::lane_id();
+  if (row >= R) return;
+  const int S = x_plan(R, D, K, tile8, grid8, F8BK).S;
+  const size_t slab_stride = (size_t)M * D;
+  float y[4];
+#pragma unroll
+  for (int k = 0; k < 4; k++) {
+    const int c = lane + 64 * k;
+    y[k] = 0.f;
+    if (c < D) {
+      const float* sp = slab + (size_t)row * D + c;
+      float sv[kMaxSplitX];
+#pragma unroll
+      for (int z = 0; z < kMaxSplitX; z++) sv[z] = sp[(z < S ? z : S - 1) * slab_stride];
+      float v = (vec || S == 1) ? sv[0] : 0.f + sv[0];
+#pragma unroll
+      for (int z = 1; z < kMaxSplitX; z++) v = z < S ? v + sv[z] : v;
+      v += b8[c];
+      y8[(size_t)row * D + c] = v;
+      y[k] = v;
+    }
+  }
+  pcnn_head::head_fwd_row(y, pw, row, D, lane, t_out, pred);
+}
+
+struct Fc8Dx {
+  int M, D, N;
+  const float* dy8;
+  int lda;
+  const float* W8;
+  int ldb;
+  const float* mask;
+  int ldm;
+  float keep;
+  float* C;
+  int ldc;
+  const int32_t* M_dev;
+};
+
+__global__ void __launch_bounds__(256, 4) k_fc8_dx_skinny(Fc8Dx a) {
+  const int Meff = eff_dim(a.M, a.M_dev);
+  const int mb = (Meff + 31) / 32, ng = (a.N + 127) / 128;
+  const int lane = pcnn::lane_id(), wave = threadIdx.x >> 6;
+  const int r = lane & 31, hsel = lane >> 5;
+  const int ns = (a.D + F8BK - 1) / F8BK;
+  const XOp oa = x_op(a.dy8, a.lda, (long)(a.M - 1) * a.lda + a.D);
+  const XOp ob = x_op(a.W8, a.ldb, (long)(a.N - 1) * a.ldb + a.D);
+  const XOp om = x_op(a.mask, a.ldm, a.mask ? (long)(a.M - 1) * a.ldm + a.N : 0);
+  const XOp oc = x_op(a.C, a.ldc, (long)(a.M - 1) * a.ldc + a.N);
+  const bool msk = a.mask != nullptr;
+  for (int item = blockIdx.x; item < mb * ng; item += gridDim.x) {
+    const int cg = item / mb, m0 = (item - cg * mb) * 32;
+    const int n0 = cg * 128 + wave * 32;
+    if (n0 >= a.N) continue;
+    const int am = m0 + r, bn = n0 + r;
+    const bool aok = am < Meff, bok = bn < a.N;
+    const unsigned abase = (unsigned)(am * a.lda + 8 * hsel) * 4u, bbase = (unsigned)(bn * a.ldb + 8 * hsel) * 4u;
+    auto load = [&](int s, xf4 (&x)[2], xf4 (&w)[2]) {
+#pragma unroll
+      for (int h = 0; h < 2; h++) {
+        const bool in = s < ns && F8BK * s + 8 * hsel + 4 * h < a.D;
+        const unsigned ko = (unsigned)(F8BK * s + 4 * h) * 4u;
+        x[h] = x_ld4(oa, in && aok ? abase + ko : kXOob, 0);
+        w[h] = x_ld4(ob, in && bok ? bbase + ko : kXOob, 0);
+      }
+    };
+    xf4 xa[2][2], xb[2][2];
+    load(0, xa[0], xb[0]);
+    const int rlane = m0 + 4 * hsel;
+    float mv[16];
+    if (msk) {
+#pragma unroll
+      for (int q = 0; q < 16; q++) {
+        const bool ok = bok && rlane + f8_qrow(q) < Meff;
+        mv[q] = x_ld1(om, ok ? (unsigned)((rlane + f8_qrow(q)) * a.ldm + bn) * 4u : kXOob, 0);
+      }
+    }
+    f32x16 acc = (f32x16){};
+#pragma unroll
+    for (int s = 0; s < F8MAXD / F8BK; s++)
+      if (s < ns) {
+        if (s + 1 < F8MAXD / F8BK) load(s + 1, xa[(s + 1) & 1], xb[(s + 1) & 1]);
+        float va[8], vb[8];
+#pragma unroll
+        for (int h = 0; h < 2; h++)
+#pragma unroll
+          for (int e = 0; e < 4; e++) {
+            va[4 * h + e] = xa[s & 1][h][e];
+            vb[4 * h + e] = xb[s & 1][h][e];
+          }
+        bf16x8 ah, am_, al, bh, bm, bl;
+        f8_split8(va, ah, am_, al);
+        f8_split8(vb, bh, bm, bl);
+        acc = f8_mfma6(ah, am_, al, bh, bm, bl, acc);
+      }
+#pragma unroll
+    for (int q = 0; q < 16; q++) {
+      const bool ok = bok && rlane + f8_qrow(q) < Meff;
+      float v = acc[q] + 0.f;
+      if (msk && !(mv[q] > 0.f)) v = 0.f;
+      if (a.keep != 1.f) v = v / a.keep;
+      __builtin_amdgcn_raw_buffer_store_b32(__builtin_bit_cast(unsigned, v), oc.rs,
+                                            ok ? (unsigned)((rlane + f8_qrow(q)) * a.ldc + bn) * 4u : kXOob, 0, 0);
+    }
+  }
+}
+
+inline LaunchPlan fc8_plan(int M, int D, int K, bool m_dynamic) { return plan_launch(M, D, K, m_dynamic, 2); }
+
+}
+
+extern "C" int pcnn_fc8_fwd_fused(int M, int N7, int K7, const void* fc7_workspace, size_t fc7_workspace_bytes,
+                                  const float* b7, int act7, float* y7, int ld7, uint8_t* drop, int ldd,
+                                  float keep_prob, int drop_gen, uint64_t seed, const int64_t* step_dev,
+                                  int stream_id, const float* W8, int ldb, int D, const int32_t* M_dev,
+                                  void* fc8_workspace, size_t fc8_workspace_bytes, void* stream) {
+  PCNN_REQUIRE(M >= 0 && N7 > 0 && K7 >= 0 && fc7_workspace && y7 && W8 && fc8_workspace);
+  PCNN_REQUIRE(D > 0 && D <= F8MAXD && ldb >= D && ld7 >= N7);
+  PCNN_REQUIRE(act7 == 0 || act7 == 1);
+  PCNN_REQUIRE(keep_prob > 0.f && keep_prob <= 1.f && (keep_prob == 1.f || drop));
+  PCNN_REQUIRE(!drop_gen || (drop && stream_id >= 0));
+  PCNN_REQUIRE(N7 % 4 == 0 && ld7 % 4 == 0 &&
+               ((((uintptr_t)fc7_workspace) | ((uintptr_t)y7) | ((uintptr_t)b7)) & 15) == 0);
+  PCNN_REQUIRE(!drop || (ldd >= N7 && ldd % 4 == 0 && ((uintptr_t)drop & 3) == 0 && (long)M * ldd < (1l << 31)));
+  PCNN_REQUIRE((long)M * ld7 < (1l << 29) && (long)N7 * ldb < (1l << 29) && (long)M * N7 < (1l << 29));
+  if (M == 0) return PCNN_OK;
+  const bool dyn = M_dev != nullptr;
+  if (fc7_workspace_bytes < gemm_workspace_bytes(M, N7, K7, dyn, 2) ||
+      fc8_workspace_bytes < gemm_workspace_bytes(M, D, N7, dyn, 2) ||
+      fc8_workspace_bytes < (size_t)M * D * sizeof(float))
+    return PCNN_ECAPACITY;
+  const LaunchPlan p7 = plan_launch(M, N7, K7, dyn, 2), p8 = fc8_plan(M, D, N7, dyn);
+  GemmArgs g{M, N7, K7, nullptr, nullptr, 0, nullptr, 0, y7, ld7, b7, act7, nullptr, 0, M_dev, nullptr,
+             (float*)fc7_workspace, 2, p7.tile, p7.grid, 0, drop, ldd, keep_prob};
+  if (drop_gen) {
+    g.drop_gen = 1;
+    g.drop_k0 = (uint32_t)seed;
+    g.drop_k1 = (uint32_t)(seed >> 32);
+    g.drop_sid = (uint32_t)stream_id;
+    g.drop_step = step_dev;
+  }
+  const Fc8Fwd a{W8, ldb, D, p8.tile, p8.grid, (float*)fc8_workspace};
+  const long items = (long)((M + 31) / 32) * kMaxSplitX;
+  const int grid = (int)(items < 512 ? items : 512);
+  hipLaunchKernelGGL(k_fc8_fwd_fused, dim3(grid), dim3(256), 0, (hipStream_t)stream, g, a);
+  PCNN_CHECK_LAUNCH();
+  return PCNN_OK;
+}
+
+extern "C" int pcnn_fc8_reduce_head_fwd(const void* fc8_workspace, size_t fc8_workspace_bytes, const float* b8,
+                                        int R_cap, int K, int D, const int32_t* num_rois_dev,
+                                        const float* poses_weight, float* y8, float* tanh_out, float* pred,
+                                        void* stream) {
+  PCNN_REQUIRE(fc8_workspace && b8 && poses_weight && y8 && tanh_out && pred && R_cap >= 0 && K >= 0);
+  PCNN_REQUIRE(D > 0 && D <= F8MAXD);
+  if (R_cap == 0) return PCNN_OK;
+  const bool dyn = num_rois_dev != nullptr;
+  if (fc8_workspace_bytes < gemm_workspace_bytes(R_cap, D, K, dyn, 2) ||
+      fc8_workspace_bytes < (size_t)R_cap * D * sizeof(float))
+    return PCNN_ECAPACITY;
+  const LaunchPlan p8 = fc8_plan(R_cap, D, K, dyn);
+  const int vec = (D & 3) == 0 && ((((uintptr_t)fc8_workspace) | ((uintptr_t)y8) | ((uintptr_t)b8)) & 15) == 0;
+  hipLaunchKernelGGL(k_fc8_reduce_head_fwd, dim3((R_cap + 3) / 4), dim3(256), 0, (hipStream_t)stream,
+                     (const float*)fc8_workspace, b8, R_cap, K, D, p8.tile, p8.grid, vec, num_rois_dev, poses_weight,
+                     y8, tanh_out, pred);
+  PCNN_CHECK_LAUNCH();
+  return PCNN_OK;
+}
+
+extern "C" int pcnn_fc8_dx_skinny(const float* dy8, int lda, const float* W8, int ldb, const float* mask, int ldm,
+                                  float keep_prob, float* dy7, int ldc, int M, int D, int N7,
+                                  const int32_t* M_dev, void* stream) {
+  PCNN_REQUIRE(dy8 && W8 && dy7 && M >= 0 && N7 > 0);
+  PCNN_REQUIRE(D > 0 && D <= F8MAXD && D % 4 == 0);
+  PCNN_REQUIRE(lda >= D && ldb >= D && ldc >= N7 && (!mask || ldm >= N7));
+  PCNN_REQUIRE(keep_prob > 0.f && keep_prob <= 1.f);
+  PCNN_REQUIRE(lda % 4 == 0 && ldb % 4 == 0 && ((((uintptr_t)dy8) | ((uintptr_t)W8)) & 15) == 0);
+  PCNN_REQUIRE((long)M * lda < (1l << 29) && (long)N7 * ldb < (1l << 29) && (long)M * ldc < (1l << 29) &&
+               (!mask || (long)M * ldm < (1l << 29)));
+  if (M == 0) return PCNN_OK;
+  const Fc8Dx a{M, D, N7, dy8, lda, W8, ldb, mask, ldm, keep_prob, dy7, ldc, M_dev};
+  const long items = (long)((M + 31) / 32) * ((N7 + 127) / 128);
+  const int grid = (int)(items < 2048 ? items : 2048);
+  pcnn::launch_last(k_fc8_dx_skinny, dim3(grid), dim3(256), 0, (hipStream_t)stream, a);
+  PCNN_CHECK_LAUNCH();
+  return PCNN_OK;
+}
diff --git a/posecnn_amd/csrc/gemm.hip b/posecnn_amd/csrc/gemm.hip
--- a/posecnn_amd/csrc/gemm.hip
+++ b/posecnn_amd/csrc/gemm.hip
@@ -96,7 +96,7 @@
                      int ldb, int b_trans, float* Cm, int ldc, const float* bias, int act, const float* mask, int ldm,
                      const uint8_t* drop, int ldd, float keep_prob, const int32_t* M_dev, const int32_t* K_dev,
                      int precision, void* workspace, size_t workspace_bytes, void* stream, int drop_gen,
-                     uint64_t seed, const int64_t* step_dev, int stream_id) {
+                     uint64_t seed, const int64_t* step_dev, int stream_id, bool skip_reduce = false) {
   PCNN_REQUIRE(M >= 0 && N > 0 && K >= 0 && A && B && Cm);
   PCNN_REQUIRE(!drop_gen || (drop && N % 4 == 0 && ldd % 4 == 0 && ((uintptr_t)drop & 3) == 0 && stream_id >= 0 &&
                              (long)M * (N / 4) < (1l << 31)));
@@ -124,7 +124,7 @@
     g.drop_step = step_dev;
   }
   hipStream_t st = (hipStream_t)stream;
-  const bool reduce_after = reduce_follows(plan, precision, drop, keep_prob);
+  const bool reduce_after = !skip_reduce && reduce_follows(plan, precision, drop, keep_prob);
   if (precision == 0) {
     launch_gemm_f32(g, a_trans, b_trans, st);
     if (reduce_after) launch_gemm_reduce(g, st);
@@ -164,3 +164,11 @@
                    keep_prob, M_dev, K_dev, precision, workspace, workspace_bytes, stream, 1, seed, step_dev,
                    stream_id);
 }
+
+extern "C" int pcnn_gemm_partial(int M, int N, int K, const float* A, const float* A2, int lda, int a_trans,
+                                 const float* B, int ldb, int b_trans, float* Cm, int ldc, const float* bias, int act,
+                                 const int32_t* M_dev, const int32_t* K_dev, int precision, void* workspace,
+                                 size_t workspace_bytes, void* stream) {
+  return gemm_impl(M, N, K, A, A2, lda, a_trans, B, ldb, b_trans, Cm, ldc, bias, act, nullptr, 0, nullptr, 0, 1.f,
+                   M_dev, K_dev, precision, workspace, workspace_bytes, stream, 0, 0, nullptr, 0, true);
+}
diff --git a/posecnn_amd/csrc/head_common.h b/posecnn_amd/csrc/head_common.h
--- a/posecnn_amd/csrc/head_common.h
+++ b/posecnn_amd/csrc/head_common.h
@@ -2,6 +2,30 @@
 #include "pcnn_common.h"
 
 namespace pcnn_head {
+
+__device__ __forceinline__ void head_fwd_row(const float (&y)[4], const float* __restrict__ pw, int row, int D,
+                                             int lane, float* __restrict__ t_out, float* __restrict__ pred) {
+  float mv[4];
+  float ss = 0.f;
+#pragma unroll
+  for (int k = 0; k < 4; k++) {
+    const int c = lane + 64 * k;
+    mv[k] = 0.f;
+    if (c < D) {
+      const float t = tanhf(y[k]);
+      t_out[(size_t)row * D + c] = t;
+      mv[k] = t * pw[(size_t)row * D + c];
+      ss += mv[k] * mv[k];
+    }
+  }
+  ss = pcnn::wave_sum(ss);
+  const float inv = 1.f / sqrtf(fmaxf(ss, 1e-12f));
+#pragma unroll
+  for (int k = 0; k < 4; k++) {
+    const int c = lane + 64 * k;
+    if (c < D) pred[(size_t)row * D + c] = mv[k] * inv;
+  }
+}
 
 __device__ __forceinline__ void head_bwd_row(const float (&dp)[4], const float* __restrict__ t_in,
                                              const float* __restrict__ pw, const float* __restrict__ pred, int row,
diff --git a/posecnn_amd/csrc/pose_head.hip b/posecnn_amd/csrc/pose_head.hip
--- a/posecnn_amd/csrc/pose_head.hip
+++ b/posecnn_amd/csrc/pose_head.hip
@@ -31,26 +31,13 @@
   const int row = (blockIdx.x * blockDim.x + threadIdx.x) >> 6;
   const int lane = pcnn::lane_id();
   if (row >= R) return;
-  float mv[4];
-  float ss = 0.f;
+  float y[4];
 #pragma unroll
   for (int k = 0; k < 4; k++) {
     const int c = lane + 64 * k;
-    mv[k] = 0.f;
-    if (c < D) {
-      const float t = tanhf(y8[(size_t)row * D + c]);
-      t_out[(size_t)row * D + c] = t;
-      mv[k] = t * pw[(size_t)row * D + c];
-      ss += mv[k] * mv[k];
-    }
+    y[k] = c < D ? y8[(size_t)row * D + c] : 0.f;
   }
-  ss = pcnn::wave_sum(ss);
-  const float inv = 1.f / sqrtf(fmaxf(ss, 1e-12f));
-#pragma unroll
-  for (int k = 0; k < 4; k++) {
-    const int c = lane + 64 * k;
-    if (c < D) pred[(size_t)row * D + c] = mv[k] * inv;
-  }
+  pcnn_head::head_fwd_row(y, pw, row, D, lane, t_out, pred);
 }
 
 __global__ void __launch_bounds__(256) k_head_bwd(const float* __restrict__ dpred, const float* __restrict__ t_in,
diff --git a/posecnn_amd/pipeline.py b/posecnn_amd/pipeline.py
--- a/posecnn_amd/pipeline.py
+++ b/posecnn_amd/pipeline.py
@@ -19,7 +19,7 @@
                  global_batch=None, batch_base=0, weights=None, dist=None, backward=True, precision=2,
                  overlap_weight_grads=True, pixel_argmax=True, keep_prob=None, drop_seed=0x5EED, side_prep=True,
                  drop_in_reduce=True, pipeline=False, prefetch_at="loss", fuse_loss_tail=True,
-                 defer_side_join=False, signal_forks=True, pool_at_tail=False):
+                 defer_side_join=False, signal_forks=True, pool_at_tail=False, fuse_fc8=True):
         self.B, self.H, self.W, self.C = B, H, W, num_classes
         self.dev = device
         self.is_train, self.skip, self.vthr, self.vper, self.margin = is_train, skip_pixels, vote_threshold, \
@@ -34,6 +34,7 @@
         self.Ch = channels
         D = 4 * num_classes
         self.D = D
+        self.fuse_fc8 = bool(fuse_fc8) and dist is None and ph.fc8_fused_ok(units, D, precision) and D % 4 == 0
         self.weights = weights or ph.PoseHeadWeights(num_classes, device, in_dim=49 * channels, units=units)
         f32 = dict(dtype=torch.float32, device=device)
         i32 = dict(dtype=torch.int32, device=device)
@@ -333,10 +334,22 @@
         if gs is not None:
             gs.send_input("w7", self.y6)
         with self._t("gemm_fc7_fc8_fwd"):
-            self._g("fc7_fwd", self.y6, w.w7, self.y7, bias=w.b7, act=1, M_dev=nr, drop=self.drop7, **dk, **g7)
-            if gs is not None:
-                gs.send_input("w8", self.y7)
-            self._g("fc8_fwd", self.y7, w.w8, self.y8, bias=w.b8, act=0, M_dev=nr)
+            if self.fuse_fc8:
+                ws7 = self._timed_gemm("fc7_fwd", lambda: ph.gemm_partial(self.y6, w.w7, self.y7, bias=w.b7, act=1,
+                                                                          M_dev=nr, precision=self.prec))
+
+                def fc8_head():
+                    ph.fc8_fwd_fused(ws7, w.units, w.b7, self.y7, w.w8, act=1, drop=self.drop7,
+                                     drop_gen=g7.get("drop_gen"), M_dev=nr, **dk)
+                    if gs is not None:
+                        gs.send_input("w8", self.y7)
+                    ph.fc8_reduce_head_fwd(w.b8, w.units, h["weight"], self.y8, self.t8, self.pred, num_rois=nr)
+                self._timed_gemm("fc8_fwd", fc8_head)
+            else:
+                self._g("fc7_fwd", self.y6, w.w7, self.y7, bias=w.b7, act=1, M_dev=nr, drop=self.drop7, **dk, **g7)
+                if gs is not None:
+                    gs.send_input("w8", self.y7)
+                self._g("fc8_fwd", self.y7, w.w8, self.y8, bias=w.b8, act=0, M_dev=nr)
         if self.prefetch_at == "loss":
             self._prefetch()
         if gen:
@@ -348,7 +361,8 @@
             self._wait("rows")
             self.norm_rows.clamp_(min=1)
         with self._t("head_add_loss_fwd"):
-            ph.head_fwd(self.y8, h["weight"], self.t8, self.pred, num_rois=nr)
+            if not self.fuse_fc8:
+                ph.head_fwd(self.y8, h["weight"], self.t8, self.pred, num_rois=nr)
             if not st["prepped"]:
                 self.add_prep(points, symmetry)
             if st["prepped"] == "side":
@@ -415,7 +429,11 @@
         dk = dict(keep_prob=self.keep) if self.keep < 1.0 else {}
         ev = self._arm_fork("fc8_dx") if side is not None else None
         with self._t("gemm_fc8_fc7_dx"):
-            self._g("fc8_dx", self.dy8, w.w8, self.dy7, b_trans=1, mask=self.y7, M_dev=nr, **dk)
+            if self.fuse_fc8:
+                self._timed_gemm("fc8_dx", lambda: ph.fc8_dx(self.dy8, w.w8, self.dy7, mask=self.y7, M_dev=nr,
+                                                             precision=self.prec, **dk))
+            else:
+                self._g("fc8_dx", self.dy8, w.w8, self.dy7, b_trans=1, mask=self.y7, M_dev=nr, **dk)
         ev = self._fork_taken(ev)
         with self._t("gemm_fc8_fc7_dw_bias"):
             weight_grads("w7", self.y6, self.dy7, CAP, w.units, w.units, fork_ev=ev)
@@ -459,14 +477,18 @@
             main.wait_stream(side)
 
     def _g(self, name, A, B, C, **kw):
+        self._timed_gemm(name, lambda: ph.gemm(A, B, C, precision=self.prec, **kw))
+        return C
+
+    def _timed_gemm(self, name, launch):
         if self.gemm_timer is None:
-            return ph.gemm(A, B, C, precision=self.prec, **kw)
+            return launch()
         e0, e1 = torch.cuda.Event(enable_timing=True), torch.cuda.Event(enable_timing=True)
         e0.record()
-        ph.gemm(A, B, C, precision=self.prec, **kw)
+        out = launch()
         e1.record()
         self.gemm_timer.setdefault(name, []).append((e0, e1))
-        return C
+        return out
 
     def step(self, inputs, next_inputs=None):
         if self.pipeline:
diff --git a/posecnn_amd/pose_head.py b/posecnn_amd/pose_head.py
--- a/posecnn_amd/pose_head.py
+++ b/posecnn_amd/pose_head.py
@@ -105,6 +105,98 @@
     _lib.check(rc, "pose_head_fwd")
 
 
+FC8_FUSED_MAX_D = 128
+
+
+def fc8_fused_ok(units, D, precision=2):
+    return precision == 2 and 0 < D <= FC8_FUSED_MAX_D and units % 4 == 0
+
+
+def gemm_partial(A, B, C, bias=None, act=0, M_dev=None, precision=2, stream=None):
+    _lib.require_gpu(A, B, C)
+    for t in (A, B, C, bias):
+        if t is not None and (t.dtype != torch.float32 or t.stride(-1) != 1):
+            raise ValueError("gemm operands must be fp32 with unit inner stride")
+    M, K = A.shape
+    N = B.shape[1]
+    lib = _lib.load()
+    ws = _lib.workspace(lib.pcnn_gemm_workspace_size(M, N, K, int(M_dev is not None), precision), C.device, "gemm",
+                        stream)
+    rc = lib.pcnn_gemm_partial(M, N, K, _lib.ptr(A), None, A.stride(0), 0, _lib.ptr(B), B.stride(0), 0, _lib.ptr(C),
+                               C.stride(0), _lib.ptr(bias), int(act), _lib.ptr(M_dev), None, int(precision),
+                               _lib.ptr(ws), ws.numel(), _lib.stream_ptr(stream))
+    _lib.check(rc, "gemm_partial")
+    return ws
+
+
+def _fc8_workspace(M, D, K, M_dev, device, stream):
+    nbytes = max(_lib.load().pcnn_gemm_workspace_size(M, D, K, int(M_dev is not None), 2), M * D * 4)
+    return _lib.workspace(nbytes, device, "fc8", stream)
+
+
+def fc8_fwd_fused(fc7_ws, K7, b7, y7, W8, act=1, drop=None, keep_prob=1.0, drop_gen=None, M_dev=None, stream=None):
+    _lib.require_gpu(fc7_ws, y7, W8)
+    M, N7 = y7.shape
+    D = W8.shape[1]
+    if drop is not None and (drop.dtype != torch.uint8 or drop.stride(-1) != 1 or not drop.is_cuda):
+        raise ValueError("fc8_fwd_fused: drop must be a uint8 device tensor with unit inner stride")
+    seed, step_dev, sid = drop_gen if drop_gen is not None else (0, None, 0)
+    if step_dev is not None and (step_dev.dtype != torch.int64 or not step_dev.is_cuda):
+        raise ValueError("fc8_fwd_fused: drop_gen's step counter must be an int64 device tensor")
+    ws8 = _fc8_workspace(M, D, N7, M_dev, y7.device, stream)
+    rc = _lib.load().pcnn_fc8_fwd_fused(M, N7, int(K7), _lib.ptr(fc7_ws), fc7_ws.numel(), _lib.ptr(b7), int(act),
+                                        _lib.ptr(y7), y7.stride(0), _lib.ptr(drop),
+                                        drop.stride(0) if drop is not None else 0, float(keep_prob),
+                                        int(drop_gen is not None), int(seed) & ((1 << 64) - 1), _lib.ptr(step_dev),
+                                        int(sid), _lib.ptr(W8), W8.stride(0), D, _lib.ptr(M_dev), _lib.ptr(ws8),
+                                        ws8.numel(), _lib.stream_ptr(stream))
+    _lib.check(rc, "fc8_fwd_fused")
+
+
+def fc8_reduce_head_fwd(b8, K, poses_weight, y8, tanh_out, pred, num_rois=None, stream=None):
+    R, D = y8.shape
+    if not (y8.is_contiguous() and tanh_out.is_contiguous() and pred.is_contiguous() and
+            poses_weight.is_contiguous()):
+        raise ValueError("fc8_reduce_head_fwd: contiguous (R, D) rows")
+    ws8 = _fc8_workspace(R, D, K, num_rois, y8.device, stream)
+    rc = _lib.load().pcnn_fc8_reduce_head_fwd(_lib.ptr(ws8), ws8.numel(), _lib.ptr(b8), R, int(K), D,
+                                              _lib.ptr(num_rois), _lib.ptr(poses_weight), _lib.ptr(y8),
+                                              _lib.ptr(tanh_out), _lib.ptr(pred), _lib.stream_ptr(stream))
+    _lib.check(rc, "fc8_reduce_head_fwd")
+
+
+def fc8_dx(dy8, W8, dy7, mask=None, keep_prob=1.0, M_dev=None, precision=2, stream=None):
+    D = W8.shape[1]
+    if not (fc8_fused_ok(W8.shape[0], D, precision) and D % 4 == 0):
+        return gemm(dy8, W8, dy7, b_trans=1, mask=mask, M_dev=M_dev, precision=precision, keep_prob=keep_prob,
+                    stream=stream)
+    _lib.require_gpu(dy8, W8, dy7, mask)
+    for t in (dy8, W8, dy7, mask):
+        if t is not None and (t.dtype != torch.float32 or t.stride(-1) != 1):
+            raise ValueError("gemm operands must be fp32 with unit inner stride")
+    rc = _lib.load().pcnn_fc8_dx_skinny(_lib.ptr(dy8), dy8.stride(0), _lib.ptr(W8), W8.stride(0), _lib.ptr(mask),
+                                        mask.stride(0) if mask is not None else 0, float(keep_prob), _lib.ptr(dy7),
+                                        dy7.stride(0), dy8.shape[0], D, W8.shape[0], _lib.ptr(M_dev),
+                                        _lib.stream_ptr(stream))
+    _lib.check(rc, "fc8_dx_skinny")
+    return dy7
+
+
+def fc7_fc8_head_fwd(y6, w7, b7, y7, w8, b8, y8, poses_weight, tanh_out, pred, drop=None, keep_prob=1.0,
+                     drop_gen=None, M_dev=None, precision=2, fuse=True, stream=None):
+    dk = dict(keep_prob=keep_prob) if keep_prob < 1.0 else {}
+    if fuse and fc8_fused_ok(w7.shape[1], w8.shape[1], precision):
+        ws7 = gemm_partial(y6, w7, y7, bias=b7, act=1, M_dev=M_dev, precision=precision, stream=stream)
+        fc8_fwd_fused(ws7, w7.shape[0], b7, y7, w8, act=1, drop=drop, drop_gen=drop_gen, M_dev=M_dev, stream=stream,
+                      **dk)
+        fc8_reduce_head_fwd(b8, w8.shape[0], poses_weight, y8, tanh_out, pred, num_rois=M_dev, stream=stream)
+        return
+    gemm(y6, w7, y7, bias=b7, act=1, M_dev=M_dev, drop=drop, drop_gen=drop_gen, precision=precision, stream=stream,
+         **dk)
+    gemm(y7, w8, y8, bias=b8, act=0, M_dev=M_dev, precision=precision, stream=stream)
+    head_fwd(y8, poses_weight, tanh_out, pred, num_rois=M_dev, stream=stream)
+
+
 def head_bwd(d_pred, tanh_out, poses_weight, pred, d_y8, num_rois=None, d_pred_scale=None, stream=None):
     R, D = d_pred.shape
     rc = _lib.load().pcnn_pose_head_bwd(_lib.ptr(d_pred), _lib.ptr(d_pred_scale), _lib.ptr(tanh_out),
```

Result: faster. 4688 (median of 6 runs) (+1.0%).
